# razayunus/ManhattanSLAM

Hardware: AMD Instinct MI355X
Metric: RGB-D frames/sec at 640x480 (ORB+surfel front end) (higher is better)
Workload: dtype u8/i32 (ORB)/f32+f64 (surfel)

## Files before the change

### manhattanslam_amd/csrc/msl_sf.h

```cpp
#pragma once

#include "msl_common.h"

#include <hip/hip_ext.h>

namespace msl {
namespace sf {

constexpr int SP = 8;
constexpr int NCHUNK = 10;
constexpr double MAX_ANGLE_COS = 0.1, HUBER_RANGE = 0.4, MIN_TOLERATE_DIFF = 0.1;
constexpr unsigned T_INF = 0xFFFFFFFFu;
constexpr int PROP_ROUNDS = 6;
constexpr unsigned short IDX_NONE = 0xFFFF, IDX_PLANE = 0xFFFE;
constexpr int LIST_D = 256;
constexpr int SCAN_ITEMS = 1024;
#ifndef MSL_SUB_ITEMS
#define MSL_SUB_ITEMS 128
#endif
constexpr int SUB_ITEMS = MSL_SUB_ITEMS;
constexpr int DEFER_WIN = 32;
#ifndef MSL_FUSEREC_PLANES
#define MSL_FUSEREC_PLANES 0
#endif
__host__ __device__ inline size_t fuserec_index(int nseeds, unsigned seed, int word) {
#if MSL_FUSEREC_PLANES
    return (size_t)word * (size_t)nseeds + seed;
#else
    (void)nseeds; return 3 * (size_t)seed + (size_t)word;
#endif
}

enum SfCtr {
    CTR_LIVE = 0,
    CTR_NEW = 1,
    CTR_DELETED = 2,
    CTR_UPDATED = 3,
    CTR_BEFORE = 4,
    CTR_ERR = 5,
    CTR_AFTER = 6,
    CTR_TAIL_FLAG = 7,
    CTR_SELECTED = 7,
    CTR_TOT_NEW = 8, CTR_TOT_DELETED = 9, CTR_TOT_UPDATED = 10, CTR_TOT_KF = 11, CTR_TOT_BEFORE = 12,
    CTR_WIDE = 13,
    CTR_COUNT = 16
};

struct alignas(16) HotPk { float px, py, pz; unsigned tl; };
struct HotRec { float px, py, pz; int updateTimes, lastUpdate; };
constexpr unsigned HOT_WIDE = 0x80000000u, HOT_HOLE = 0xFFFFFFFFu;
__host__ __device__ inline bool tl_fits(int ut, int lu) { return (unsigned)ut < 2048u && ((unsigned)lu + (1u << 19)) < (1u << 20); }
__host__ __device__ inline unsigned tl_pack(int ut, int lu) { return ((unsigned)ut << 20) | ((unsigned)lu & 0xFFFFFu); }
__host__ __device__ inline int tl_ut(unsigned tl) { return (int)(tl >> 20); }
__host__ __device__ inline int tl_lu(unsigned tl) { return (int)(tl << 12) >> 12; }
struct alignas(32) ColdRec { float nx, ny, nz, size, color, weight; unsigned rgbf; unsigned _spare; };
constexpr unsigned COLD_WIDE = 1u << 24;
struct MapSoA {
    HotPk *hot;
    ColdRec *cold;
    int *rgbWide;
    int *utlWide;
    long long *wideFlag;
};
__host__ __device__ inline bool rgb_fits(int r, int g, int b) { return ((unsigned)r | (unsigned)g | (unsigned)b) < 256u; }
__host__ __device__ inline unsigned rgb_pack(int r, int g, int b) { return (unsigned)r | ((unsigned)g << 8) | ((unsigned)b << 16); }

template <typename T> using gptr = const T __attribute__((address_space(1))) *;
struct FrameDev {
    const uint8_t *gray; const float *depth; const int32_t *member;
    float pose[16], invPose[16];
    int ref, _pad;
#ifdef __HIPCC__
    __device__ __forceinline__ gptr<uint8_t> grayG() const { return (gptr<uint8_t>)gray; }
    __device__ __forceinline__ gptr<float> depthG() const { return (gptr<float>)depth; }
    __device__ __forceinline__ gptr<int32_t> memberG() const { return (gptr<int32_t>)member; }
#endif
};

struct alignas(32) AssignRec {
    float x, y, meanIntensity;
    unsigned stable;
    double invDepth;
    unsigned long long _pad;
};

struct FuseAux {
    MapSoA map;
    unsigned long long cap;
    unsigned *delU, *delUCount;
    unsigned *delList;
};
struct DeferCtl {
    long long ext[DEFER_WIN + 1];
    unsigned delCnt[DEFER_WIN];
    unsigned logBase[DEFER_WIN];
    unsigned nMoves;
    int flagStride;
    const uint8_t *candOk, *fused;
    const msl_surfel *cand;
    FuseAux aux;
};

struct SfDev {
    int W, H, spW, spH, nseeds, npx;
    float fx, fy, cx, cy, fuseFar, fuseNear;
    unsigned long long gstride, gbytes, dstride, mstride;
    unsigned gsB, dsB, msB;
    const FrameDev *frames;
    msl_seed *seeds, *seedsTmp;
    msl_surfel *cand;
    uint8_t *candOk;
    uint8_t *fused;
    uint2 *tex;
    float4 *fuseRec;
    unsigned short *index, *amap;
    unsigned *tmin;
    AssignRec *arec;
    float *pxInv;
    unsigned *wl;
    unsigned *wlCount;
    int *chunkAbort;
    int *changed;
    MapSoA map;
    unsigned long long cap;
    long long *ctr;
    msl_surfel *newSurfels;
    unsigned *blockSums, *blockUpd, *delList, *srcOf;
    unsigned *sbKeys, *deal;
    int dealG;
    unsigned *tickets;
    unsigned *delU;
    unsigned *delUCount;
    const float *colX, *rowY;
    int pxStride;
    int flagStride;
    int kf;
    int prevSlotAbs;
    DeferCtl *dc;
    unsigned *moveDst;
    unsigned long long *loc64;
    unsigned *vposD;
    unsigned *locKeys, *vposKeys;
    unsigned *dBig;
    unsigned *bitmap;
    HotPk *stageHot; ColdRec *stageCold; int *stageRgb, *stageUtl;
};

#ifdef __HIPCC__
__device__ __forceinline__ AssignRec assign_rec(const msl_seed &s) {
    AssignRec a;
    a.x = s.x; a.y = s.y; a.meanIntensity = s.meanIntensity; a.stable = s.stable ? 1u : 0u;
    a.invDepth = s.meanDepth > 0 ? 1.0 / (double)s.meanDepth : -1.0; a._pad = 0;
    return a;
}
__device__ __forceinline__ int seed_chunk(int seedI, int nseeds) {
    const int step = nseeds / NCHUNK;
    if (step == 0) return NCHUNK - 1;
    const int c = seedI / step;
    return c > NCHUNK - 1 ? NCHUNK - 1 : c;
}
template <typename T> __device__ __forceinline__ gptr<T> byte_off(gptr<T> p, unsigned off) {
    return reinterpret_cast<gptr<T>>(reinterpret_cast<const char __attribute__((address_space(1))) *>(p) + off);
}
template <typename T> __device__ __forceinline__ gptr<T> byte_off(const T *p, unsigned off) { return byte_off((gptr<T>)p, off); }
template <typename T> using gptr_w = T __attribute__((address_space(1))) *;
template <typename T> __device__ __forceinline__ gptr_w<T> byte_off_w(T *p, unsigned off) {
    return reinterpret_cast<gptr_w<T>>(reinterpret_cast<char __attribute__((address_space(1))) *>((gptr_w<T>)p) + off);
}
__device__ __forceinline__ uint8_t gray_at(const SfDev &P, const FrameDev &F, int y, int x) { return *byte_off(F.grayG(), (unsigned)y * P.gsB + (unsigned)x); }
__device__ __forceinline__ float depth_at(const SfDev &P, const FrameDev &F, int y, int x) { return *byte_off(F.depthG(), (unsigned)y * P.dsB + 4u * (unsigned)x); }
__device__ __forceinline__ int32_t member_at(const SfDev &P, const FrameDev &F, int y, int x) {
    return *byte_off(F.memberG(), ((unsigned)y >> 1) * P.msB + 4u * ((unsigned)x >> 1));
}
__device__ __forceinline__ void vec3b(const SfDev &P, const FrameDev &F, float row, float col, int &r, int &g, int &b) {
    const unsigned long long off = (unsigned long long)(int)row * P.gstride + 3ull * (unsigned long long)(int)col;
    r = off < P.gbytes ? F.grayG()[off] : 0;
    g = off + 1 < P.gbytes ? F.grayG()[off + 1] : 0;
    b = off + 2 < P.gbytes ? F.grayG()[off + 2] : 0;
}
__device__ __forceinline__ void back_project(const SfDev &P, float u, float v, float d, float &x, float &y, float &z) {
    x = (u - P.cx) / P.fx * d;
    y = (v - P.cy) / P.fy * d;
    z = d;
}
__device__ __forceinline__ float get_weight(float d) { const double a = 1.0 / (double)d / (double)d; return (float)(1.0 < a ? 1.0 : a); }
__device__ __forceinline__ void mul4(const float *m, float v0, float v1, float v2, float v3, float out[4]) {
#pragma unroll
    for (int r = 0; r < 4; r++) out[r] = ((m[r] * v0 + m[4 + r] * v1) + m[8 + r] * v2) + m[12 + r] * v3;
}
__device__ __forceinline__ void mul3(const float *m, float v0, float v1, float v2, float out[3]) {
#pragma unroll
    for (int r = 0; r < 3; r++) out[r] = (m[r] * v0 + m[4 + r] * v1) + m[8 + r] * v2;
}
#endif

template <typename T>
__host__ __device__ inline void inverse4(const T *m, T *inv) {
#define M_(r, c) m[(c) * 4 + (r)]
#define DET3(r0, r1, r2, c0, c1, c2)                                                                     \
    (M_(r0, c0) * (M_(r1, c1) * M_(r2, c2) - M_(r1, c2) * M_(r2, c1)) -                                 \
     M_(r0, c1) * (M_(r1, c0) * M_(r2, c2) - M_(r1, c2) * M_(r2, c0)) +                                 \
     M_(r0, c2) * (M_(r1, c0) * M_(r2, c1) - M_(r1, c1) * M_(r2, c0)))
    T cof[4][4];
    for (int r = 0; r < 4; r++)
        for (int c = 0; c < 4; c++) {
            int rr[3], cc[3], k = 0;
            for (int i = 0; i < 4; i++) if (i != r) rr[k++] = i;
            k = 0;
            for (int i = 0; i < 4; i++) if (i != c) cc[k++] = i;
            const T d = DET3(rr[0], rr[1], rr[2], cc[0], cc[1], cc[2]);
            cof[r][c] = ((r + c) & 1) ? -d : d;
        }
    const T det = ((M_(0, 0) * cof[0][0] + M_(0, 1) * cof[0][1]) + M_(0, 2) * cof[0][2]) + M_(0, 3) * cof[0][3];
    for (int r = 0; r < 4; r++)
        for (int c = 0; c < 4; c++) inv[c * 4 + r] = cof[c][r] / det;
#undef DET3
#undef M_
}

#ifdef __HIPCC__
__device__ __forceinline__ bool xcd_slot(int blocksPerFrame, int nSlots, int &slot, int &blk) {
    const unsigned lin = blockIdx.x;
    const unsigned j = lin >> 3;
    slot = (int)(lin & 7u) + 8 * (int)(j / (unsigned)blocksPerFrame);
    blk = (int)(j % (unsigned)blocksPerFrame);
    return slot < nSlots;
}
#endif
inline unsigned xcd_grid(int blocksPerFrame, int nSlots) { return 8u * (unsigned)((nSlots + 7) / 8) * (unsigned)blocksPerFrame; }

enum { SK_SEED_INIT = 0, SK_ASSIGN, SK_PROP, SK_COMMIT_PX, SK_UPDATE_SEEDS, SK_COMMIT_SEEDS, SK_SEED_PLANE, SK_FUSE, SK_NEW, SK_COMPACT,
       SK_CONVERT, SK_COPY };

#define MSL_SF_LAUNCH_LDS(prof, kid, st, kern, grid, block, lds, ...)                                  \
    do {                                                                                               \
        hipEvent_t _ea, _eb;                                                                           \
        if ((prof).kernel_pair(kid, &_ea, &_eb))                                                       \
            hipExtLaunchKernelGGL(kern, grid, block, lds, st, _ea, _eb, 0, __VA_ARGS__);               \
        else                                                                                           \
            hipLaunchKernelGGL(kern, grid, block, lds, st, __VA_ARGS__);                               \
    } while (0)
#define MSL_SF_LAUNCH(prof, kid, st, kern, grid, block, ...) MSL_SF_LAUNCH_LDS(prof, kid, st, kern, grid, block, 0, __VA_ARGS__)

bool sp_init_attributes(int nseeds);
void sp_launch_stage(KernelProfiler &prof, hipStream_t st, const SfDev &P, int nFrames, bool propLds);
void sp_launch_depth_u16(hipStream_t st, const void *src, size_t srcStride, size_t srcFrameStride, float *dst, size_t dstFrameStride, int W, int H, int nFrames,
                         float factor);
int sp_debug_div100(const float *x_host, double *out_host, size_t n);
int sp_debug_chain(const float *x_host, const int32_t *n_host, int lists, int huber, float *out_host);
void map_launch_fuse(KernelProfiler &prof, hipStream_t st, const SfDev &P, int slot, const FrameDev &F, int nSubGrid, int nSubHint, bool deferred, bool dealt, unsigned blkStride);
void map_launch_compact(KernelProfiler &prof, hipStream_t st, const SfDev &P, int slot, bool resident);
void map_launch_deal(hipStream_t st, const SfDev &P);
int map_debug_deal(const uint32_t *keys_host, int G, uint32_t *deal_host);
void map_launch_replay(KernelProfiler &prof, hipStream_t st, const SfDev &P, int nFrames, unsigned blkStride);
void map_launch_empty_pair(KernelProfiler &prof, hipStream_t st);
void map_launch_set_ctr(hipStream_t st, const SfDev &P, long long n, int wide);
void map_launch_add_ctr(hipStream_t st, const SfDev &P, long long add);
void map_launch_aos_to_soa(KernelProfiler &prof, hipStream_t st, const SfDev &P, const msl_surfel *src, long long n, bool atEnd);
void map_launch_soa_to_aos(KernelProfiler &prof, hipStream_t st, const SfDev &P, msl_surfel *dst, long long n);
void map_launch_select_count(hipStream_t st, const SfDev &P, int mode, int arg);
void map_launch_select_write(hipStream_t st, const SfDev &P, int mode, int arg, msl_surfel *out, int markDeleted);
void map_launch_collect_changed(hipStream_t st, const SfDev &P, int ref, long long n, unsigned *count, unsigned *idxOut, msl_surfel *recOut, unsigned capOut);
void map_launch_empty(hipStream_t st, int grid, hipEvent_t a, hipEvent_t b);

}
}
```

### manhattanslam_amd/csrc/msl_sf_compact.hip

```cpp

#include "msl_sf_map_dev.h"

namespace {
template <int NT>
__device__ __forceinline__ void deal_subblocks(const unsigned *keys, int G, unsigned *deal, unsigned *s_hist, unsigned *s_off, unsigned *s_wave, unsigned *s_aux) {
    static_assert(NT == 256, "one histogram bin per thread");
    const unsigned t = threadIdx.x;
    constexpr int CH = 32 * NT;
    auto load_pack = [&](int base, unsigned (&kp)[8]) {
        uint4 v[8];
#pragma unroll
        for (int q = 0; q < 8; q++) v[q] = *reinterpret_cast<const uint4 *>(keys + base + 32 * (int)t + 4 * q);
#pragma unroll
        for (int q = 0; q < 8; q++) kp[q] = min(v[q].x, 255u) | (min(v[q].y, 255u) << 8) | (min(v[q].z, 255u) << 16) | (min(v[q].w, 255u) << 24);
    };
    auto next_word = [&](unsigned (&kp)[8]) -> unsigned {
        const unsigned w = kp[0];
#pragma unroll
        for (int q = 0; q < 7; q++) kp[q] = kp[q + 1];
        kp[7] = w;
        return w;
    };
    auto count_chunk = [&](int base, unsigned (&kp)[8], bool hist) -> unsigned {
        unsigned fc = 0;
#pragma unroll 1
        for (int d = 0; d < 8; d++) {
            const unsigned w = next_word(kp);
#pragma unroll
            for (int b = 0; b < 4; b++) {
                const unsigned key = (w >> (8 * b)) & 255u;
                const bool in = base + 32 * (int)t + 4 * d + b < G;
                if (hist && in && key != 255u) atomicAdd(&s_hist[key], 1u);
                fc += in && key == 255u ? 1u : 0u;
            }
        }
        return fc;
    };
    unsigned k0[8];
    load_pack(0, k0);
    s_hist[t] = 0;
    __syncthreads();
    const unsigned fc0 = count_chunk(0, k0, true);
    for (int base = CH; base < G; base += CH) { unsigned kc[8]; load_pack(base, kc); (void)count_chunk(base, kc, true); }
    __syncthreads();
    unsigned NI, fTot0, ex, fb0;
    block_excl_scan_pair(t < 255u ? s_hist[t] : 0u, fc0, s_wave, &NI, &fTot0, ex, fb0);
    const unsigned gs = (unsigned)G >> 3;
    auto inS = [&](unsigned x) { return (x * NI + 7u) >> 3; };
    auto outS = [&](unsigned x) { return x * gs - inS(x); };
    {
        unsigned x0 = 0;
#pragma unroll
        for (unsigned y = 1; y < 8; y++) x0 += ex >= inS(y) ? 1u : 0u;
        s_off[t] = ex - inS(x0);
        s_hist[t] = x0 | ((inS(x0 + 1) - inS(x0)) << 3);
        if (t < 9) s_aux[t] = inS(t);
    }
    __syncthreads();
    unsigned fillBase = 0;
    auto place_chunk = [&](int base, unsigned (&kp)[8], unsigned fb, unsigned ftot) {
        fb += fillBase;
        fillBase += ftot;
        unsigned xf = 0;
#pragma unroll
        for (unsigned y = 1; y < 8; y++) xf += fb >= outS(y) ? 1u : 0u;
        unsigned jf = (inS(xf + 1) - inS(xf)) + (fb - outS(xf));
#pragma unroll 1
        for (int d = 0; d < 8; d++) {
            const unsigned w = next_word(kp);
            unsigned rr[4], tb[4];
#pragma unroll
            for (int b = 0; b < 4; b++) {
                const unsigned key = (w >> (8 * b)) & 255u;
                rr[b] = 0; tb[b] = 0;
                if (base + 32 * (int)t + 4 * d + b < G && key != 255u) { rr[b] = atomicAdd(&s_off[key], 1u); tb[b] = s_hist[key]; }
            }
#pragma unroll
            for (int b = 0; b < 4; b++) {
                const unsigned key = (w >> (8 * b)) & 255u;
                const int sb = base + 32 * (int)t + 4 * d + b;
                const bool in = sb < G, iv = in && key != 255u, fl = in && key == 255u;
                unsigned x = tb[b] & 7u, room = tb[b] >> 3, j = rr[b];
                if (__builtin_expect(__ballot((iv && j >= room) || (fl && jf >= gs)) != 0ull, 0)) {
                    if (iv) while (j >= room) { j -= room; x++; room = s_aux[x + 1] - s_aux[x]; }
                    if (fl) while (jf >= gs) { xf++; jf = s_aux[xf + 1] - s_aux[xf]; }
                }
                const unsigned at = (iv ? x : xf) * gs + (iv ? j : jf);
                if (in) deal[at] = (unsigned)sb;
                jf += fl ? 1u : 0u;
            }
        }
    };
    place_chunk(0, k0, fb0, fTot0);
    for (int base = CH; base < G; base += CH) {
        unsigned kc[8];
        load_pack(base, kc);
        const unsigned fc = count_chunk(base, kc, false);
        unsigned ftot;
        const unsigned fb = block_excl_scan(fc, s_wave, &ftot);
        place_chunk(base, kc, fb, ftot);
    }
    __syncthreads();
}
__global__ __launch_bounds__(256) void k_deal(const unsigned *keys, int G, unsigned *deal) {
    __shared__ unsigned s_hist[256], s_off[256], s_wave[33], s_aux[16];
    deal_subblocks<256>(keys, G, deal, s_hist, s_off, s_wave, s_aux);
}

constexpr int TAIL_MAX_HOPS = 64;


constexpr int SMALL_D = 512, SMALL_CHUNKS = 48;

struct CompactArgs {
    int nseeds, flagStride, dealG, _pad;
    unsigned long long cap;
    MapSoA map;
    long long *ctr;
    const uint8_t *candOk, *fused;
    const msl_surfel *cand;
    msl_surfel *newSurfels;
    unsigned *blockSums, *blockUpd, *delList, *srcOf, *tickets, *delU, *delUCount;
    const unsigned *sbKeys; unsigned *deal;
};
__host__ inline CompactArgs compact_args(const SfDev &P, int slot) {
    CompactArgs A;
    A.nseeds = P.nseeds; A.flagStride = P.flagStride; A.dealG = P.dealG; A._pad = 0; A.cap = P.cap; A.map = P.map; A.ctr = P.ctr;
    A.candOk = P.candOk + (size_t)slot * P.flagStride; A.fused = P.fused + (size_t)slot * P.flagStride; A.cand = P.cand + (size_t)slot * P.nseeds;
    A.newSurfels = P.newSurfels; A.blockSums = P.blockSums; A.blockUpd = P.blockUpd; A.delList = P.delList; A.srcOf = P.srcOf; A.tickets = P.tickets;
    A.delU = P.delU; A.delUCount = P.delUCount; A.sbKeys = P.sbKeys; A.deal = P.deal;
    return A;
}

template <int NQW>
__global__ __launch_bounds__(256) void k_compact(CompactArgs P, int mode) {
    constexpr int NT = 256, TILE = 4 * NT;
    __shared__ unsigned s_wave[33];
    __shared__ unsigned s_dl[SMALL_D];
    __shared__ unsigned s_raw[LIST_D];
    __shared__ unsigned s_last, s_upd, s_nzChunks, s_base, s_cntChunk;
    __shared__ unsigned s_nzIdx[SMALL_CHUNKS], s_nzCnt[SMALL_CHUNKS], s_nzSortIdx[SMALL_CHUNKS], s_nzSortCnt[SMALL_CHUNKS];
    __shared__ int s_fallback;
    __builtin_amdgcn_s_setprio(3);
    if (mode == 0 && blockIdx.x == 1 && P.dealG > 0) deal_subblocks<NT>(P.sbKeys, P.dealG, P.deal, s_raw, s_dl, s_wave, s_nzIdx);
    if (mode == 0 && blockIdx.x != 0 && *P.delUCount <= LIST_D) return;
    const uint4 bs0 = *reinterpret_cast<const uint4 *>(P.blockSums + 4 * threadIdx.x);
    constexpr int NBU = 8;
    uint4 bu[NBU];
#pragma unroll
    for (int q = 0; q < NBU; q++) bu[q] = *reinterpret_cast<const uint4 *>(P.blockUpd + TILE * q + 4 * threadIdx.x);
    static_assert(LIST_D == NT, "one hand-over entry per thread");
    const unsigned du = P.delU[threadIdx.x];
    const unsigned dHand = *P.delUCount;
    const long long n = P.ctr[CTR_LIVE];
    const bool bad = P.ctr[CTR_ERR] == 20;
    const uint8_t *candOk = P.candOk, *fused = P.fused;
    const int per = (((P.nseeds + NT - 1) / NT) + 3) & ~3;
    const int s0 = threadIdx.x * per, s1 = min(s0 + per, P.nseeds);
    unsigned cnt = 0;
    unsigned long long emit = 0, emitHi = 0;
    const msl_surfel *cand = P.cand;
    const bool aligned4 = (P.nseeds & 3) == 0 && ((reinterpret_cast<size_t>(candOk) | reinterpret_cast<size_t>(fused)) & 3) == 0;
    auto flags_in_one_trip = [&](auto nqTag) {
        constexpr int NQ = decltype(nqTag)::value;
        unsigned cw[NQ], fw[NQ];
#pragma unroll
        for (int q = 0; q < NQ; q++) {
            const int i = s0 + 4 * q;
            const bool in = 4 * q < per && i < s1;
            cw[q] = in ? *reinterpret_cast<const unsigned *>(candOk + i) : 0u;
            fw[q] = in ? *reinterpret_cast<const unsigned *>(fused + i) : 0u;
        }
#pragma unroll
        for (int q = 0; q < NQ; q += 8)
            asm volatile("" ::"v"(cw[q]), "v"(cw[q + 1]), "v"(cw[q + 2]), "v"(cw[q + 3]), "v"(cw[q + 4]), "v"(cw[q + 5]), "v"(cw[q + 6]), "v"(cw[q + 7]),
                         "v"(fw[q]), "v"(fw[q + 1]), "v"(fw[q + 2]), "v"(fw[q + 3]), "v"(fw[q + 4]), "v"(fw[q + 5]), "v"(fw[q + 6]), "v"(fw[q + 7]));
#pragma unroll
        for (int q = 0; q < NQ; q++)
#pragma unroll
            for (int j = 0; j < 4; j++) {
                const unsigned e = (s0 + 4 * q + j < s1 && ((cw[q] >> (8 * j)) & 0xFF) && !((fw[q] >> (8 * j)) & 0xFF)) ? 1u : 0u;
                cnt += e;
                if (4 * q + j < 64) emit |= (unsigned long long)e << ((4 * q + j) & 63);
                else emitHi |= (unsigned long long)e << ((4 * q + j - 64) & 63);
            }
    };
    if constexpr (NQW > 0) {
        (void)aligned4;
        flags_in_one_trip(std::integral_constant<int, NQW>{});
    } else {
        for (int i = s0; i < s1; i += 4) {
            unsigned c4, f4;
            if (i + 4 <= P.nseeds && ((reinterpret_cast<size_t>(candOk + i) | reinterpret_cast<size_t>(fused + i)) & 3) == 0) {
                c4 = *reinterpret_cast<const unsigned *>(candOk + i); f4 = *reinterpret_cast<const unsigned *>(fused + i);
            } else {
                c4 = f4 = 0;
                for (int j = 0; j < 4 && i + j < P.nseeds; j++) { c4 |= (unsigned)candOk[i + j] << (8 * j); f4 |= (unsigned)fused[i + j] << (8 * j); }
            }
#pragma unroll
            for (int j = 0; j < 4; j++) {
                const unsigned e = (i + j < s1 && ((c4 >> (8 * j)) & 0xFF) && !((f4 >> (8 * j)) & 0xFF)) ? 1u : 0u;
                cnt += e;
                if (i + j - s0 < 64) emit |= (unsigned long long)e << (i + j - s0);
                else if (i + j - s0 < 128) emitHi |= (unsigned long long)e << (i + j - s0 - 64);
            }
        }
    }
    const long long nblk = (n + SUB_ITEMS - 1) / SUB_ITEMS;
    const long long nWg = nblk;
    unsigned updPart = 0;
#pragma unroll
    for (int q = 0; q < NBU; q++) {
        const long long c = TILE * q + 4 * threadIdx.x;
        updPart += (c < nWg ? bu[q].x : 0u) + (c + 1 < nWg ? bu[q].y : 0u) + (c + 2 < nWg ? bu[q].z : 0u) + (c + 3 < nWg ? bu[q].w : 0u);
    }
    s_raw[threadIdx.x] = du;
    if (threadIdx.x == 0) { s_upd = 0; s_fallback = 0; s_nzChunks = 0; }
    __syncthreads();
    const bool fastest = mode == 0 && dHand <= LIST_D;
    unsigned vsum = 0;
    if (!fastest)
        for (long long t0 = 0; t0 < nblk; t0 += TILE) {
            const long long c = t0 + 4 * threadIdx.x;
            const uint4 v4 = t0 == 0 ? bs0 : *reinterpret_cast<const uint4 *>(P.blockSums + c);
            const unsigned x[4] = {c < nblk ? v4.x : 0u, c + 1 < nblk ? v4.y : 0u, c + 2 < nblk ? v4.z : 0u, c + 3 < nblk ? v4.w : 0u};
#pragma unroll
            for (int j = 0; j < 4; j++)
                if (x[j] > 0) {
                    vsum += x[j];
                    const unsigned q = atomicAdd(&s_nzChunks, 1u);
                    if (q < SMALL_CHUNKS) { s_nzIdx[q] = (unsigned)(c + j); s_nzCnt[q] = x[j]; }
                }
        }
    unsigned Dtot, Ku, exUnused, pos;
    block_excl_scan_pair(vsum, cnt, s_wave, &Dtot, &Ku, exUnused, pos);
    const long long D = fastest ? (long long)dHand : (long long)Dtot;
    const bool small = mode == 0 && !fastest && D <= SMALL_D && s_nzChunks <= SMALL_CHUNKS;
    const bool single = fastest || small;
    if (single && blockIdx.x != 0) return;
    if (mode == 0 && !bad) {
        if (fastest) {
            if (threadIdx.x < D) {
                unsigned r = 0;
                for (unsigned j = 0; j < (unsigned)D; j++) r += s_raw[j] < du ? 1u : 0u;
                s_dl[r] = du;
            }
        } else if (small) {
            const unsigned nz = s_nzChunks;
            if (threadIdx.x < nz) {
                const unsigned me = s_nzIdx[threadIdx.x];
                unsigned r = 0;
                for (unsigned j = 0; j < nz; j++) r += s_nzIdx[j] < me ? 1u : 0u;
                s_nzSortIdx[r] = me; s_nzSortCnt[r] = s_nzCnt[threadIdx.x];
            }
            __syncthreads();
            unsigned base = 0;
            for (unsigned it = 0; it < nz; it++) {
                const long long i0 = (long long)s_nzSortIdx[it] * SUB_ITEMS + threadIdx.x;
                const unsigned f = (threadIdx.x < (unsigned)SUB_ITEMS && i0 < n && hot_is_deleted(P.map, i0)) ? 1u : 0u;
                unsigned tt;
                const unsigned w = base + block_excl_scan(f, s_wave, &tt);
                if (f) s_dl[w] = (unsigned)i0;
                base += s_nzSortCnt[it];
            }
        } else {
            unsigned carry = 0;
            for (long long t0 = 0; t0 < nblk; t0 += TILE) {
                const long long c = t0 + 4 * threadIdx.x;
                const uint4 v4 = t0 == 0 ? bs0 : *reinterpret_cast<const uint4 *>(P.blockSums + c);
                const unsigned v[4] = {c < nblk ? v4.x : 0u, c + 1 < nblk ? v4.y : 0u, c + 2 < nblk ? v4.z : 0u, c + 3 < nblk ? v4.w : 0u};
                unsigned tot;
                const unsigned ex = carry + block_excl_scan(v[0] + v[1] + v[2] + v[3], s_wave, &tot);
                const long long nIter = (min(t0 + TILE, nblk) - t0 - blockIdx.x + gridDim.x - 1) / gridDim.x;
                for (long long it = 0; it < nIter; it++) {
                    const long long b = t0 + blockIdx.x + it * gridDim.x;
                    const int q = (int)(b - t0);
                    if ((int)threadIdx.x == (q >> 2)) {
                        const int comp = q & 3;
                        s_base = ex + (comp > 0 ? v[0] : 0u) + (comp > 1 ? v[1] : 0u) + (comp > 2 ? v[2] : 0u);
                        s_cntChunk = v[comp];
                    }
                    __syncthreads();
                    const unsigned base = s_base, cntChunk = s_cntChunk;
                    if (cntChunk == 0) { __syncthreads(); continue; }
                    const long long i0 = b * SUB_ITEMS + threadIdx.x;
                    const unsigned f = (threadIdx.x < (unsigned)SUB_ITEMS && i0 < n && hot_is_deleted(P.map, i0)) ? 1u : 0u;
                    unsigned tt;
                    const unsigned w = base + block_excl_scan(f, s_wave, &tt);
                    if (f) st_agent(&P.delList[w], (unsigned)i0);
                }
                carry += tot;
                __syncthreads();
            }
        }
    }
    __syncthreads();
    if (mode == 0 && !single && !last_workgroup(&P.tickets[1], &s_last)) return;
    {
        unsigned u = updPart;
        for (long long c2 = (long long)NBU * TILE + threadIdx.x; c2 < nWg; c2 += blockDim.x) u += P.blockUpd[c2];
        u = wave_incl_scan(u);
        if ((threadIdx.x & 63) == 63 && u) atomicAdd(&s_upd, u);
    }
    const long long K = Ku;
    const long long nAfter = mode == 1 ? n : (D >= K ? n - (D - K) : n + (K - D));
    const bool place = mode == 0 && !bad && (unsigned long long)nAfter <= P.cap;
    auto DL = [&](long long j) -> unsigned { return single ? s_dl[j] : ld_agent(&P.delList[j]); };
    if (cnt) {
        auto emit_one = [&](const msl_surfel &e) {
            const long long k = pos++;
            P.newSurfels[k] = e;
            if (place)
                store_surfel(P.map, k < D ? (long long)DL(D - 1 - k) : n + (k - D), e);
        };
        for (unsigned long long m = emit; m; m &= m - 1) emit_one(cand[s0 + __builtin_ctzll(m)]);
        for (unsigned long long mh = emitHi; mh; mh &= mh - 1) emit_one(cand[s0 + 64 + __builtin_ctzll(mh)]);
        for (int i = s0 + 128; i < s1; i++)
            if (candOk[i] && !fused[i]) emit_one(cand[i]);
    }
    __syncthreads();
    if (threadIdx.x == 0) {
        P.ctr[CTR_NEW] = K; P.ctr[CTR_DELETED] = D; P.ctr[CTR_UPDATED] = s_upd; P.ctr[CTR_BEFORE] = n; P.ctr[CTR_AFTER] = nAfter;
        P.ctr[CTR_TOT_NEW] += K; P.ctr[CTR_TOT_DELETED] += D; P.ctr[CTR_TOT_UPDATED] += s_upd; P.ctr[CTR_TOT_KF] += 1; P.ctr[CTR_TOT_BEFORE] += n;
        if ((unsigned long long)nAfter > P.cap) P.ctr[CTR_ERR] = 20;
    }
    if (!place) { if (threadIdx.x == 0) *P.delUCount = 0; return; }
    const long long t0 = threadIdx.x, stride = blockDim.x;
    if (D > K) {
        const long long R = D - K, nFinal = n - R;
        auto lower = [&](long long x) -> long long {
            long long lo = 0, hi = R;
            while (lo < hi) { const long long mid = (lo + hi) >> 1; if ((long long)DL(mid) < x) lo = mid + 1; else hi = mid; }
            return lo;
        };
        const long long cntLow = lower(nFinal);
        for (long long a = t0; a < cntLow; a += stride) {
            long long p = nFinal + a;
            int hop = 0;
            for (; hop < TAIL_MAX_HOPS; hop++) {
                const long long lb = lower(p);
                if (lb < R && (long long)DL(lb) == p) p = n - (R - lb);
                else break;
            }
            if (hop == TAIL_MAX_HOPS) s_fallback = 1;
            P.srcOf[a] = (unsigned)p;
        }
        __syncthreads();
        if (s_fallback) {
            if (threadIdx.x == 0)
                for (long long i = 1; i <= R; i++) {
                    const long long hole = DL(R - i), src = n - i;
                    if (src != hole) move_surfel(P.map, hole, src);
                }
        } else {
            for (long long a = t0; a < cntLow; a += stride) move_surfel(P.map, (long long)DL(a), (long long)P.srcOf[a]);
        }
    }
    if (threadIdx.x == 0) { P.ctr[CTR_LIVE] = nAfter; *P.delUCount = 0; }
}
}

namespace msl {
namespace sf {
void map_launch_compact(KernelProfiler &prof, hipStream_t st, const SfDev &P, int slot, bool resident) {
    const CompactArgs A = compact_args(P, slot);
    const int per = (((P.nseeds + 255) / 256) + 3) & ~3;
    const bool aligned4 = (P.nseeds & 3) == 0 && ((reinterpret_cast<size_t>(A.candOk) | reinterpret_cast<size_t>(A.fused)) & 3) == 0;
    const dim3 grid(resident ? 128 : 1);
    if (per <= 32 && aligned4) MSL_SF_LAUNCH(prof, SK_COMPACT, st, k_compact<8>, grid, dim3(256), A, resident ? 0 : 1);
    else if (per <= 96 && aligned4) MSL_SF_LAUNCH(prof, SK_COMPACT, st, k_compact<24>, grid, dim3(256), A, resident ? 0 : 1);
    else MSL_SF_LAUNCH(prof, SK_COMPACT, st, k_compact<0>, grid, dim3(256), A, resident ? 0 : 1);
}
void map_launch_deal(hipStream_t st, const SfDev &P) { hipLaunchKernelGGL(k_deal, dim3(1), dim3(256), 0, st, P.sbKeys, P.dealG, P.deal); }
int map_debug_deal(const uint32_t *keys_host, int G, uint32_t *deal_host) {
    if (!keys_host || !deal_host || G < 8 || (G & 7)) return MSL_ERR_INVALID;
    const size_t pad = (size_t)G + 8192;
    DevBuf keys, deal;
    MSL_HIP_TRY(grow_all(0, {{keys, sizeof(unsigned) * pad}, {deal, sizeof(unsigned) * (G + 64)}}));
    unsigned *dk = (unsigned *)keys.p, *dd = (unsigned *)deal.p;
    MSL_HIP_TRY(hipMemset(dk, 0xFF, sizeof(unsigned) * pad)); MSL_HIP_TRY(hipMemset(dd, 0xFF, sizeof(unsigned) * G));
    MSL_HIP_TRY(hipMemcpy(dk, keys_host, sizeof(unsigned) * G, hipMemcpyHostToDevice));
    hipLaunchKernelGGL(k_deal, dim3(1), dim3(256), 0, 0, dk, G, dd);
    MSL_HIP_TRY(hipGetLastError());
    MSL_HIP_TRY(hipMemcpy(deal_host, dd, sizeof(unsigned) * G, hipMemcpyDeviceToHost));
    return MSL_OK;
}
}
}
```

### manhattanslam_amd/csrc/msl_sf_debug.hip

```cpp

#include "msl_sf_handle.h"

#include <vector>

using namespace msl;
using namespace msl::sf;

namespace {
const char *kSfNames[MSL_SF_NKERNELS] = {"kb_seed_init", "kb_assign", "kb_prop", "kb_commit_px", "kb_update_seeds", "kb_commit_seeds",
                                         "kb_seed_plane", "k_fuse", "k_empty", "k_compact", "k_convert", "copy"};
}

extern "C" {

int msl_sf_debug_seeds(msl_sf *h, msl_seed *out) noexcept {
    try {
    if (!h || !out) return MSL_ERR_INVALID;
    MSL_HIP_TRY(hipSetDevice(h->device));
    int rc = sync_all(h);
    if (rc != MSL_OK) return rc;
    const size_t ns = h->dev.nseeds;
    MSL_HIP_TRY(hipMemcpy(out, h->dev.seeds + ns * h->lastSlot, sizeof(msl_seed) * ns, hipMemcpyDeviceToHost));
    std::vector<uint8_t> fused(ns);
    MSL_HIP_TRY(hipMemcpy(fused.data(), h->dev.fused + (size_t)h->dev.flagStride * h->lastSlot, ns, hipMemcpyDeviceToHost));
    for (size_t i = 0; i < ns; i++) out[i].fused = fused[i] & 1;
    return MSL_OK;
    } MSL_ABI_CATCH_INT
}
int msl_sf_debug_ctr(msl_sf *h, int64_t out[16]) noexcept {
    try {
    if (!h || !out) return MSL_ERR_INVALID;
    MSL_HIP_TRY(hipSetDevice(h->device));
    int rc = read_ctr(h);
    if (rc != MSL_OK) return rc;
    static_assert(CTR_COUNT == 16, "msl_sf_debug_ctr hands out every counter");
    for (int i = 0; i < CTR_COUNT; i++) out[i] = host_ctr(h, (SfCtr)i);
    return MSL_OK;
    } MSL_ABI_CATCH_INT
}
int msl_sf_debug_scratch(msl_sf *h, int which, size_t offset_words, uint32_t *out, size_t n_words) noexcept {
    try {
    if (!h || !out || which < 0 || which > 5) return MSL_ERR_INVALID;
    if (which == 5) {
        if (n_words < 2) return MSL_ERR_INVALID;
        out[0] = (uint32_t)h->kfClassic; out[1] = (uint32_t)h->kfDeferred;
        return MSL_OK;
    }
    if (which == 4) {
        if (n_words < 1) return MSL_ERR_INVALID;
        out[0] = (uint32_t)h->dealG;
        return MSL_OK;
    }
    if (offset_words + n_words > (which < 2 ? h->dev.cap : h->blkStride)) return MSL_ERR_INVALID;
    MSL_HIP_TRY(hipSetDevice(h->device));
    int rc = sync_all(h);
    if (rc != MSL_OK) return rc;
    const uint32_t *src = which == 0 ? h->dev.srcOf : which == 1 ? h->dev.delList : which == 2 ? h->dev.sbKeys : h->dev.deal;
    MSL_HIP_TRY(hipMemcpy(out, src + offset_words, sizeof(uint32_t) * n_words, hipMemcpyDeviceToHost));
    return MSL_OK;
    } MSL_ABI_CATCH_INT
}
int msl_sf_debug_event_overhead(msl_sf *h, int grid, int n, float *mean_us) noexcept {
    try {
    if (!h || !mean_us || n < 1 || grid < 1) return MSL_ERR_INVALID;
    MSL_HIP_TRY(hipSetDevice(h->device));
    int rc = sync_all(h);
    if (rc != MSL_OK) return rc;
    std::vector<hipEvent_t> ev(2 * (size_t)n);
    for (auto &e : ev) MSL_HIP_TRY(hipEventCreate(&e));
    for (int i = 0; i < n; i++) map_launch_empty(h->mapStream, grid, ev[2 * i], ev[2 * i + 1]);
    MSL_HIP_TRY(hipStreamSynchronize(h->mapStream));
    double tot = 0;
    for (int i = 0; i < n; i++) { float ms = 0; MSL_HIP_TRY(hipEventElapsedTime(&ms, ev[2 * i], ev[2 * i + 1])); tot += ms; }
    for (auto &e : ev) (void)hipEventDestroy(e);
    *mean_us = (float)(tot * 1e3 / n);
    return MSL_OK;
    } MSL_ABI_CATCH_INT
}
int msl_sf_debug_index(msl_sf *h, int32_t *out) noexcept {
    try {
    if (!h || !out) return MSL_ERR_INVALID;
    MSL_HIP_TRY(hipSetDevice(h->device));
    int rc = sync_all(h);
    if (rc != MSL_OK) return rc;
    const size_t npx = h->dev.npx;
    std::vector<unsigned short> tmp(npx);
    MSL_HIP_TRY(hipMemcpy(tmp.data(), h->dev.index + (size_t)h->dev.pxStride * h->lastSlot, sizeof(unsigned short) * npx, hipMemcpyDeviceToHost));
    for (size_t i = 0; i < npx; i++) out[i] = tmp[i];
    return MSL_OK;
    } MSL_ABI_CATCH_INT
}

int msl_debug_deal(const uint32_t *keys_host, int n_subblocks, uint32_t *deal_host) noexcept { try { return map_debug_deal(keys_host, n_subblocks, deal_host); } MSL_ABI_CATCH_INT }
int msl_debug_div100(const float *x_host, double *out_host, size_t n) noexcept { try { return sp_debug_div100(x_host, out_host, n); } MSL_ABI_CATCH_INT }
int msl_debug_chain_sum(const float *x_host, const int32_t *n_host, int lists, int huber, float *out_host) noexcept { try { return sp_debug_chain(x_host, n_host, lists, huber, out_host); } MSL_ABI_CATCH_INT }
const char *msl_sf_kernel_name(int k) noexcept { try { return (k >= 0 && k < MSL_SF_NKERNELS) ? kSfNames[k] : ""; } MSL_ABI_CATCH_PTR }

}
```

### manhattanslam_amd/csrc/msl_sf_fuse.hip

```cpp

#include "msl_sf_map_dev.h"

namespace {
__device__ __forceinline__ void mul4r(const float *m, float v0, float v1, float v2, float v3, float out[3]) {
#pragma unroll
    for (int r = 0; r < 3; r++) out[r] = ((m[r] * v0 + m[3 + r] * v1) + m[6 + r] * v2) + m[9 + r] * v3;
}
__device__ __forceinline__ void mul3r(const float *m, float v0, float v1, float v2, float out[3]) {
#pragma unroll
    for (int r = 0; r < 3; r++) out[r] = (m[r] * v0 + m[3 + r] * v1) + m[6 + r] * v2;
}

template <bool DEFER, bool spawnWave>
__device__ __forceinline__ void fuse_body(const FuseArgs &P, const FuseFrame &F, int nSubHint, unsigned waveIdx, int G) {
    constexpr int KPL = SUB_ITEMS / 64;
    constexpr long long WSPAN = 64 * KPL;
    struct { HotPk *hot; ColdRec *cold; } M = {P.hot, P.cold};
    const FuseAux *aux = &P.dc->aux;
    const unsigned lane0 = threadIdx.x;
    const uint2 *tex = P.tex;
    const float4 *fuseRec = P.fuseRec;
    uint8_t *fused = P.fused;
    const int ref = F.ref;
    const float cameraF = (float)(((double)fabsf(P.fx) + (double)fabsf(P.fy)) / 2.0);
    const float halfF = 0.5f * cameraF;
    const bool pending = DEFER && P.kf > 0;
    long long E0v = 0;
    if (pending) E0v = P.dc->ext[P.kf - 1];
    long long E0 = 0;
    if (DEFER && spawnWave) E0 = ((long long)__builtin_amdgcn_readfirstlane((int)(E0v >> 32)) << 32) | (unsigned)__builtin_amdgcn_readfirstlane((int)E0v);
    if (spawnWave && !pending) return;
    if (DEFER && !pending && waveIdx == 0 && lane0 == 0) P.dc->ext[0] = P.ctr[CTR_LIVE];
    if (DEFER && !spawnWave && waveIdx == 0 && lane0 == 0) P.dc->logBase[P.kf] = P.kf > 0 ? P.dc->logBase[P.kf - 1] + P.dc->delCnt[P.kf - 1] : 0u;
    unsigned spK = 0;
    if (DEFER && spawnWave) {
        unsigned excl;
        spK = spawn_count(P, lane0, excl);
        if (lane0 == 0) P.dc->ext[P.kf] = E0 + (long long)spK;
        if (spK == 0) return;
    }
#ifndef MSL_FUSE_CHUNK
#define MSL_FUSE_CHUNK 16
#endif
    constexpr unsigned FUSE_CHUNK = MSL_FUSE_CHUNK;
    long long sb0;
    if (!spawnWave && P.deal != nullptr) {
        const unsigned gs = (unsigned)G >> 3;
        const unsigned *dp = P.deal + ((waveIdx & 7u) * gs + (waveIdx >> 3));
        unsigned dv;
        asm volatile("s_load_dword %0, %1, 0x0\n\ts_waitcnt lgkmcnt(0)" : "=s"(dv) : "s"(dp) : "memory");
        sb0 = (long long)dv;
    } else {
        long long lin = waveIdx;
        constexpr unsigned T = 8u * FUSE_CHUNK;
        const unsigned full = ((unsigned)G / T) * T;
        if (waveIdx < full) { const unsigned grp = waveIdx / T, r = waveIdx % T; lin = (long long)grp * T + (r & 7u) * FUSE_CHUNK + (r >> 3); }
        sb0 = (long long)G - 1 - lin;
    }
    for (long long it = 0;; it++) {
        unsigned lane = lane0;
        asm volatile("" : "+v"(lane));
#define REC_LOCAL(k) (64u * (unsigned)(k) + lane)
        const long long sb = sb0 + it * G;
        long long c0, n = 0, cntIdx;
        if (DEFER && spawnWave) {
            c0 = E0 + it * WSPAN;
            n = E0 + (long long)spK;
            if (c0 >= n) return;
            unsigned excl;
            (void)spawn_count(P, lane, excl);
            emit_records(P, E0, c0, KPL, lane, spK, excl);
            cntIdx = E0 / SUB_ITEMS + 1 + it;
        } else {
            c0 = sb * WSPAN; cntIdx = sb;
            if (pending) {
                if (it > 0) {
                    E0 = ((long long)__builtin_amdgcn_readfirstlane((int)(E0v >> 32)) << 32) | (unsigned)__builtin_amdgcn_readfirstlane((int)E0v);
                    if (c0 >= E0) return;
                }
            } else if (sb >= nSubHint && c0 >= __hip_atomic_load(&P.ctr[CTR_LIVE], __ATOMIC_RELAXED, __HIP_MEMORY_SCOPE_AGENT)) return;
        }
        HotPk hq[KPL];
#pragma unroll
        for (int k = 0; k < KPL; k++) hq[k] = M.hot[c0 + REC_LOCAL(k)];
        if (!pending) n = P.ctr[CTR_LIVE];
        else if (!spawnWave) {
            E0 = ((long long)__builtin_amdgcn_readfirstlane((int)(E0v >> 32)) << 32) | (unsigned)__builtin_amdgcn_readfirstlane((int)E0v);
            if (c0 >= E0) return;
            n = E0;
        }
        unsigned stp = 0;
        unsigned keyAcc = 0;
        float pzv[KPL];
        unsigned offT[KPL];
        unsigned anyTl = 0;
#pragma unroll
        for (int k = 0; k < KPL; k++) anyTl |= hq[k].tl;
        const bool anyHi = __builtin_expect(__ballot(anyTl >> 31) != 0ull, 0);
#pragma unroll
        for (int k = 0; k < KPL; k++) {
            const long long i = c0 + REC_LOCAL(k);
            const float x = hq[k].px, y = hq[k].py, z = hq[k].pz;
            const unsigned tl = hq[k].tl;
            int ut = tl_ut(tl), lu = tl_lu(tl);
            bool hole = false;
            if (anyHi) {
                if (tl == HOT_WIDE) { const int *w = aux->map.utlWide; ut = w[2 * i]; lu = w[2 * i + 1]; }
                else if (tl & 0x80000000u) hole = true;
            }
            float pc[3];
            mul4r(F.inv, x, y, z, 1.0f, pc);
            const bool inRange = !(pc[2] < P.fuseNear || pc[2] > P.fuseFar);
            const bool live = i < n && !hole, stale = ref - lu > 5 && ut < 5;
            int st = 0;
            if (live) st = stale ? (ut != 0 ? 1 : 2) : (ut == 0 ? 2 : 0);
            const bool cand = live && !stale && ut != 0 && inRange;
            unsigned off = 0;
            {
                const float zq = inRange ? pc[2] : 1.0f;
                const float projectU = pc[0] * P.fx / zq + P.cx, projectV = pc[1] * P.fy / zq + P.cy;
                const int pUInt = round_half_up_pixel(projectU), pVInt = round_half_up_pixel(projectV);
                const bool inImage = !(pUInt < 1 || pUInt > P.W - 2 || pVInt < 1 || pVInt > P.H - 2);
                if (cand && inImage) { st = 3; keyAcc += (((unsigned)pVInt * (unsigned)P.rowScale) >> 16) | 0x10000u; }
                off = st == 3 ? (unsigned)(pVInt * P.W + pUInt) : 0u;
            }
            stp |= (unsigned)st << (2 * k); pzv[k] = pc[2];
            offT[k] = off;
        }
        uint2 tx[KPL];
        {
#pragma unroll
            for (int k = 0; k < KPL; k++) tx[k] = tex[offT[k]];
            if constexpr (KPL == 4) asm volatile("" ::"v"(tx[0].x), "v"(tx[1].x), "v"(tx[2].x), "v"(tx[3].x), "v"(tx[0].y), "v"(tx[1].y), "v"(tx[2].y), "v"(tx[3].y));
            else asm volatile("" ::"v"(tx[0].x), "v"(tx[KPL - 1].x), "v"(tx[0].y), "v"(tx[KPL - 1].y));
        }
        if (!(DEFER && spawnWave)) {
            const unsigned ks = (unsigned)__builtin_amdgcn_readlane((int)wave_incl_scan(keyAcc), 63);
            const unsigned kc = ks >> 16;
            const unsigned key = kc ? min((unsigned)((float)(ks & 0xFFFFu) * __builtin_amdgcn_rcpf((float)kc)), 254u) : 255u;
            if (lane == 0) P.sbKeys[cntIdx] = key;
        }
        unsigned fl = 0;
        unsigned cntDel = 0;
#pragma unroll
        for (int k = 0; k < KPL; k++) {
            const unsigned st = (stp >> (2 * k)) & 3u;
            const bool occluded = st == 3u && (double)pzv[k] < (double)__uint_as_float(tx[k].x) - 1.0;
            const bool del = st == 1u || st == 2u || occluded;
            if (DEFER) { if (del) M.hot[c0 + REC_LOCAL(k)].tl = HOT_HOLE; }
            else if (st == 1u || occluded) {
                if (__builtin_expect(hq[k].tl == HOT_WIDE, 0)) aux->map.utlWide[2 * (c0 + REC_LOCAL(k))] = 0;
                else M.hot[c0 + REC_LOCAL(k)].tl = hq[k].tl & 0xFFFFFu;
            }
            fl |= del ? (1u << k) : 0u;
            fl |= (st == 3u && !occluded) ? (16u << k) : 0u;
            cntDel += (unsigned)__popcll(__ballot(del));
        }
        auto list_base = [&](unsigned c) -> unsigned {
            unsigned base = 0, prior = 0;
            if (DEFER && P.kf > 0) prior = P.dc->logBase[P.kf - 1] + P.dc->delCnt[P.kf - 1];
            if (lane == 0) base = atomicAdd(P.delCount, c);
            return (unsigned)__builtin_amdgcn_readfirstlane((int)base) + prior;
        };
        auto hand_over = [&](bool d, unsigned long long m, unsigned base, long long i) {
            if (d) {
                const unsigned j = base + lane_rank(m);
                if (DEFER || j < (unsigned)LIST_D) P.delOut[j] = (unsigned)i;
            }
        };
        if (cntDel) {
            unsigned base = list_base(cntDel);
#pragma unroll
            for (int k = 0; k < KPL; k++) {
                const bool d = (fl >> k) & 1u;
                const unsigned long long m = __ballot(d);
                hand_over(d, m, base, c0 + REC_LOCAL(k)); base += (unsigned)__popcll(m);
            }
        }
        unsigned rcv[KPL], bk[KPL];
        unsigned total = 0;
#pragma unroll
        for (int k = 0; k < KPL; k++) {
            const bool sv = (fl >> (4 + k)) & 1u;
            const unsigned long long m = __ballot(sv);
            const unsigned c = (unsigned)__popcll(m), rs = lane_rank(m);
            const unsigned dest = (sv ? total + rs : total + c + (lane - rs)) & 63u;
            const unsigned payload = sv ? (REC_LOCAL(k) | 0x100u | (tx[k].y << 16)) : 0u;
            rcv[k] = (unsigned)__builtin_amdgcn_ds_permute((int)(dest * 4u), (int)payload);
            bk[k] = total;
            total += c;
        }
        const unsigned rounds = (total + 63u) >> 6;
        unsigned nupd = 0, cntDelB = 0;
        for (unsigned r = 0; r < rounds; r++) {
            unsigned item = 0u;
#pragma unroll
            for (int k = 0; k < KPL; k++) {
                const unsigned rk = (bk[k] + ((lane - bk[k]) & 63u)) >> 6;
                if ((rcv[k] & 0x100u) && rk == r) item = rcv[k];
            }
            const long long i = c0 + (item & 0xFFu);
            const unsigned sp = item >> 16;
            const HotPk h = M.hot[i];
            ColdRec c;
            {
                const float4 cn = *reinterpret_cast<const float4 *>(M.cold + i);
                c.nx = cn.x; c.ny = cn.y; c.nz = cn.z; c.size = cn.w; c.weight = M.cold[i].weight;
            }
            const float4 f0 = fuseRec[fuserec_index(P.nseeds, sp, 0)], f1 = fuseRec[fuserec_index(P.nseeds, sp, 1)], f2 = fuseRec[fuserec_index(P.nseeds, sp, 2)];
            const float *poseM = F.frame->pose;
            const float r00 = poseM[0], r10 = poseM[1], r20 = poseM[2], r01 = poseM[4], r11 = poseM[5], r21 = poseM[6], r02 = poseM[8], r12 = poseM[9], r22 = poseM[10];
            asm volatile("" ::"v"(h.px), "v"(h.tl), "v"(c.nx), "v"(c.weight), "v"(f0.x), "v"(f1.x), "v"(f2.x), "v"(r00), "v"(r01), "v"(r02));
            bool upd = false, delB = false;
            if (item && __float_as_uint(f2.w) != 0u) {
                const float seedDepth = f0.w;
                const float pz = ((F.inv[2] * h.px + F.inv[5] * h.py) + F.inv[8] * h.pz) + F.inv[11] * 1.0f;
                float tolerateDiff = (pz * pz) / halfF * 4.0f;
                tolerateDiff = tolerateDiff < MIN_TOLERATE_DIFF ? (float)MIN_TOLERATE_DIFF : tolerateDiff;
                if (!(pz < seedDepth - tolerateDiff) && !(pz > seedDepth + tolerateDiff)) {
                    float nc[3];
                    mul3r(F.inv, c.nx, c.ny, c.nz, nc);
                    const float normDiffCos = nc[0] * f0.x + nc[1] * f0.y + nc[2] * f0.z;
                    if (normDiffCos < MAX_ANGLE_COS) {
                        if (DEFER) M.hot[i].tl = HOT_HOLE;
                        else if (__builtin_expect(h.tl == HOT_WIDE, 0)) aux->map.utlWide[2 * i] = 0;
                        else M.hot[i].tl = h.tl & 0xFFFFFu;
                        delB = true;
                    } else {
                        const float oldWeight = c.weight;
                        const float newWeight = f1.w;
                        const float sumWeight = oldWeight + newWeight;
                        const float fusedPx = (h.px * oldWeight + newWeight * f1.x) / sumWeight;
                        const float fusedPy = (h.py * oldWeight + newWeight * f1.y) / sumWeight;
                        const float fusedPz = (h.pz * oldWeight + newWeight * f1.z) / sumWeight;
                        float fusedNx = nc[0] * oldWeight + newWeight * f0.x;
                        float fusedNy = nc[1] * oldWeight + newWeight * f0.y;
                        float fusedNz = nc[2] * oldWeight + newWeight * f0.z;
                        const float newNormLength = sqrtf(fusedNx * fusedNx + fusedNy * fusedNy + fusedNz * fusedNz);
                        fusedNx = fusedNx / newNormLength; fusedNy = fusedNy / newNormLength; fusedNz = fusedNz / newNormLength;
                        float newNormW[3];
                        newNormW[0] = (r00 * fusedNx + r01 * fusedNy) + r02 * fusedNz;
                        newNormW[1] = (r10 * fusedNx + r11 * fusedNy) + r12 * fusedNz;
                        newNormW[2] = (r20 * fusedNx + r21 * fusedNy) + r22 * fusedNz;
                        int ut = (int)(h.tl >> 20);
                        if (__builtin_expect(h.tl == HOT_WIDE, 0)) ut = aux->map.utlWide[2 * i];
                        unsigned tlNew = tl_pack(ut + 1, ref);
                        if (__builtin_expect(!tl_fits(ut + 1, ref), 0)) {
                            int *w = aux->map.utlWide;
                            w[2 * i] = ut + 1; w[2 * i + 1] = ref;
                            asm volatile("" ::: "memory");
                            set_wide_flag_ptr(aux->map.wideFlag, 2ull);
                            tlNew = HOT_WIDE;
                        }
                        c.rgbf = __float_as_uint(f2.z);
                        c.nx = newNormW[0]; c.ny = newNormW[1]; c.nz = newNormW[2];
                        c.weight = sumWeight;
                        c.color = f2.y;
                        const float newSize = f2.x;
                        if (newSize < c.size) c.size = newSize;
                        u32x4 hv = {__float_as_uint(fusedPx), __float_as_uint(fusedPy), __float_as_uint(fusedPz), tlNew};
                        u32x4 c0v = {__float_as_uint(c.nx), __float_as_uint(c.ny), __float_as_uint(c.nz), __float_as_uint(c.size)};
                        u32x4 c1v = {__float_as_uint(c.color), __float_as_uint(c.weight), c.rgbf, 0u};
                        st16(M.hot + i, hv);
                        st16(M.cold + i, c0v);
                        st16(reinterpret_cast<u32x4 *>(M.cold + i) + 1, c1v);
                        fused[sp] = 1;
                        upd = true;
                    }
                }
            }
            nupd += (unsigned)__popcll(__ballot(upd));
            const unsigned long long mb = __ballot(delB);
            if (mb) {
                const unsigned cb = (unsigned)__popcll(mb);
                hand_over(delB, mb, list_base(cb), i);
                cntDelB += cb;
            }
        }
        if (lane == 0) {
            if (!DEFER) P.blockSums[cntIdx] = cntDel + cntDelB;
            P.blockUpd[cntIdx] = nupd;
        }
        if (!(DEFER && spawnWave) && (sb + G) * WSPAN >= n) return;
    }
#undef REC_LOCAL
}

template <bool DEFER>
__global__ __launch_bounds__(64) __attribute__((amdgpu_waves_per_eu(6, 8))) void k_fuse(FuseArgs P, FuseFrame F, int nSubHint) {
    __builtin_amdgcn_s_setprio(3);
    if (DEFER) {
        if (blockIdx.x == 0) fuse_body<DEFER, true>(P, F, nSubHint, 0u, (int)gridDim.x - 1);
        else fuse_body<DEFER, false>(P, F, nSubHint, blockIdx.x - 1u, (int)gridDim.x - 1);
    } else {
        fuse_body<false, false>(P, F, nSubHint, blockIdx.x, (int)gridDim.x);
    }
}
}

namespace msl {
namespace sf {
void map_launch_fuse(KernelProfiler &prof, hipStream_t st, const SfDev &P, int slot, const FrameDev &F, int nSubGrid, int nSubHint, bool deferred, bool dealt, unsigned blkStride) {
    const FuseArgs A = fuse_args(P, slot, deferred, blkStride, dealt);
    const FuseFrame FF = fuse_frame(F, P.frames + slot);
    if (deferred) MSL_SF_LAUNCH(prof, SK_FUSE, st, k_fuse<true>, dim3((unsigned)nSubGrid + 1u), dim3(64), A, FF, nSubHint);
    else MSL_SF_LAUNCH(prof, SK_FUSE, st, k_fuse<false>, dim3((unsigned)nSubGrid), dim3(64), A, FF, nSubHint);
}
}
}
```

### manhattanslam_amd/csrc/msl_sf_map.hip

```cpp

#include "msl_sf_map_dev.h"

namespace {
__device__ __forceinline__ bool select_pred(const HotRec &h, int mode, int arg) {
    return mode == 0 ? (h.updateTimes > 0 && h.lastUpdate == arg) : (h.updateTimes >= arg);
}
__global__ __launch_bounds__(256) void k_select_count(SfDev P, int mode, int arg) {
    __shared__ unsigned s_c;
    const long long n = P.ctr[CTR_LIVE];
    const long long nblk = (n + SCAN_ITEMS - 1) / SCAN_ITEMS;
    for (long long b = blockIdx.x; b < nblk; b += gridDim.x) {
        if (threadIdx.x == 0) s_c = 0;
        __syncthreads();
        unsigned c = 0;
        for (int k = 0; k < SCAN_ITEMS / 256; k++) {
            const long long i = b * SCAN_ITEMS + k * 256 + threadIdx.x;
            if (i < n && select_pred(hot_load(P.map, i), mode, arg)) c++;
        }
        if (c) atomicAdd(&s_c, c);
        __syncthreads();
        if (threadIdx.x == 0) P.blockSums[b] = s_c;
        __syncthreads();
    }
}
__global__ __launch_bounds__(1024) void k_select_scan(SfDev P) {
    __shared__ unsigned s_wave[17];
    const long long n = P.ctr[CTR_LIVE];
    const int nblk = (int)((n + SCAN_ITEMS - 1) / SCAN_ITEMS);
    unsigned carry = 0;
    for (int b0 = 0; b0 < nblk; b0 += 1024) {
        const int b = b0 + threadIdx.x;
        const unsigned v = b < nblk ? P.blockSums[b] : 0;
        unsigned tot;
        const unsigned ex = carry + block_excl_scan(v, s_wave, &tot);
        if (b < nblk) P.blockSums[b] = ex;
        carry += tot;
    }
    if (threadIdx.x == 0) P.ctr[CTR_SELECTED] = carry;
}
__global__ __launch_bounds__(256) void k_select_write(SfDev P, int mode, int arg, msl_surfel *out, int markDeleted) {
    __shared__ unsigned s_wave[17];
    const long long n = P.ctr[CTR_LIVE];
    const long long nblk = (n + SCAN_ITEMS - 1) / SCAN_ITEMS;
    for (long long b = blockIdx.x; b < nblk; b += gridDim.x) {
        unsigned base = P.blockSums[b];
        for (int k = 0; k < SCAN_ITEMS / 256; k++) {
            const long long i = b * SCAN_ITEMS + k * 256 + threadIdx.x;
            HotRec h{};
            unsigned tl = 0;
            if (i < n) { tl = P.map.hot[i].tl; h = hot_load(P.map, i); }
            const bool sel = i < n && select_pred(h, mode, arg);
            unsigned tot;
            const unsigned pos = base + block_excl_scan(sel ? 1u : 0u, s_wave, &tot);
            if (sel) {
                msl_surfel e;
                load_surfel(P.map, i, h, e);
                out[pos] = e;
                if (markDeleted) hot_mark_deleted(P.map, i, tl);
            }
            base += tot;
        }
    }
}
__global__ void k_add_ctr(long long *ctr, long long add) {
    if (threadIdx.x == 0) { ctr[CTR_LIVE] += add; ctr[CTR_BEFORE] = ctr[CTR_LIVE]; ctr[CTR_AFTER] = ctr[CTR_LIVE]; }
}
__global__ __launch_bounds__(256) void k_aos_to_soa_at(MapSoA M, const msl_surfel *src, long long n, const long long *ctr) {
    const long long i = (long long)blockIdx.x * 256 + threadIdx.x;
    if (i < n) store_surfel(M, ctr[CTR_LIVE] + i, src[i]);
}

__global__ __launch_bounds__(256) void k_aos_to_soa(MapSoA M, const msl_surfel *src, long long n) {
    const long long i = (long long)blockIdx.x * 256 + threadIdx.x;
    if (i < n) store_surfel(M, i, src[i]);
}
__global__ __launch_bounds__(256) void k_soa_to_aos(MapSoA M, msl_surfel *dst, long long n) {
    const long long i = (long long)blockIdx.x * 256 + threadIdx.x;
    if (i >= n) return;
    const HotRec h = hot_load(M, i);
    msl_surfel e;
    load_surfel(M, i, h, e);
    dst[i] = e;
}
__global__ void k_set_ctr(long long *ctr, long long n, unsigned *delUCount, int wide) {
    if (threadIdx.x == 0) {
        delUCount[0] = 0;
        ctr[CTR_LIVE] = n; ctr[CTR_NEW] = 0; ctr[CTR_DELETED] = 0; ctr[CTR_UPDATED] = 0; ctr[CTR_BEFORE] = n; ctr[CTR_AFTER] = n; ctr[CTR_TAIL_FLAG] = 0;
        if (wide >= 0) ctr[CTR_WIDE] = wide;
    }
}

__global__ __launch_bounds__(64) void k_collect_changed(SfDev P, int ref, long long n, unsigned *count, unsigned *idxOut, msl_surfel *recOut, unsigned capOut) {
    const long long sb = blockIdx.x;
    if (!(P.blockSums[sb] | P.blockUpd[sb])) return;
    const unsigned lane = threadIdx.x;
    for (int k = 0; k < SUB_ITEMS / 64; k++) {
        const long long i = sb * SUB_ITEMS + k * 64 + lane;
        HotRec h; h.px = h.py = h.pz = 0; h.updateTimes = 1; h.lastUpdate = ref - 1;
        if (i < n) h = hot_load(P.map, i);
        const bool ch = i < n && (h.updateTimes == 0 || h.lastUpdate == ref);
        const unsigned long long m = __ballot(ch);
        if (!m) continue;
        unsigned base = 0;
        if (lane == 0) base = atomicAdd(count, (unsigned)__popcll(m));
        base = __builtin_amdgcn_readfirstlane(base);
        if (ch) {
            const unsigned j = base + lane_rank(m);
            if (j < capOut) { msl_surfel e; load_surfel(P.map, i, h, e); recOut[j] = e; idxOut[j] = (unsigned)i; }
        }
    }
}

__global__ void k_empty(int grid_dummy) { (void)grid_dummy; }
}

namespace msl {
namespace sf {
void map_launch_empty_pair(KernelProfiler &prof, hipStream_t st) {
    hipEvent_t ea, eb;
    if (prof.kernel_pair(SK_NEW, &ea, &eb)) hipExtLaunchKernelGGL(k_empty, dim3(1), dim3(64), 0, st, ea, eb, 0, 0);
}
void map_launch_set_ctr(hipStream_t st, const SfDev &P, long long n, int wide) { hipLaunchKernelGGL(k_set_ctr, dim3(1), dim3(64), 0, st, P.ctr, n, P.delUCount, wide); }
void map_launch_add_ctr(hipStream_t st, const SfDev &P, long long add) { hipLaunchKernelGGL(k_add_ctr, dim3(1), dim3(64), 0, st, P.ctr, add); }
void map_launch_aos_to_soa(KernelProfiler &prof, hipStream_t st, const SfDev &P, const msl_surfel *src, long long n, bool atEnd) {
    if (atEnd) hipLaunchKernelGGL(k_aos_to_soa_at, dim3((unsigned)((n + 255) / 256)), dim3(256), 0, st, P.map, src, n, P.ctr);
    else MSL_SF_LAUNCH(prof, SK_CONVERT, st, k_aos_to_soa, dim3((unsigned)((n + 255) / 256)), dim3(256), P.map, src, n);
}
void map_launch_soa_to_aos(KernelProfiler &prof, hipStream_t st, const SfDev &P, msl_surfel *dst, long long n) {
    MSL_SF_LAUNCH(prof, SK_CONVERT, st, k_soa_to_aos, dim3((unsigned)((n + 255) / 256)), dim3(256), P.map, dst, n);
}
void map_launch_select_count(hipStream_t st, const SfDev &P, int mode, int arg) {
    hipLaunchKernelGGL(k_select_count, dim3(512), dim3(256), 0, st, P, mode, arg);
    hipLaunchKernelGGL(k_select_scan, dim3(1), dim3(1024), 0, st, P);
}
void map_launch_select_write(hipStream_t st, const SfDev &P, int mode, int arg, msl_surfel *out, int markDeleted) {
    hipLaunchKernelGGL(k_select_write, dim3(512), dim3(256), 0, st, P, mode, arg, out, markDeleted);
}
void map_launch_collect_changed(hipStream_t st, const SfDev &P, int ref, long long n, unsigned *count, unsigned *idxOut, msl_surfel *recOut, unsigned capOut) {
    const unsigned nblk = (unsigned)((n + SUB_ITEMS - 1) / SUB_ITEMS);
    hipLaunchKernelGGL(k_collect_changed, dim3(nblk), dim3(64), 0, st, P, ref, n, count, idxOut, recOut, capOut);
}
void map_launch_empty(hipStream_t st, int grid, hipEvent_t a, hipEvent_t b) { hipExtLaunchKernelGGL(k_empty, dim3((unsigned)grid), dim3(64), 0, st, a, b, 0, grid); }
}
}
```

### manhattanslam_amd/csrc/msl_sf_map_dev.h

```cpp
#pragma once

#include "msl_sf.h"

#ifdef __HIPCC__

using namespace msl;
using namespace msl::sf;

namespace {

__device__ __forceinline__ unsigned ld_agent(const unsigned *p) { return __hip_atomic_load(p, __ATOMIC_RELAXED, __HIP_MEMORY_SCOPE_AGENT); }
__device__ __forceinline__ void st_agent(unsigned *p, unsigned v) { __hip_atomic_store(p, v, __ATOMIC_RELAXED, __HIP_MEMORY_SCOPE_AGENT); }
__device__ __forceinline__ unsigned long long ld_agent64(const unsigned long long *p) { return __hip_atomic_load(p, __ATOMIC_RELAXED, __HIP_MEMORY_SCOPE_AGENT); }
__device__ __forceinline__ void st_agent64(unsigned long long *p, unsigned long long v) { __hip_atomic_store(p, v, __ATOMIC_RELAXED, __HIP_MEMORY_SCOPE_AGENT); }

__device__ __forceinline__ void set_wide_flag_ptr(long long *flag, unsigned long long bit) { atomicOr(reinterpret_cast<unsigned long long *>(flag), bit); }
__device__ __forceinline__ void set_wide_flag(const MapSoA &M, unsigned long long bit) { set_wide_flag_ptr(M.wideFlag, bit); }
__device__ __forceinline__ void tl_unpack(const MapSoA &M, long long i, unsigned tl, int &ut, int &lu) {
    ut = tl_ut(tl); lu = tl_lu(tl);
    if (tl & 0x80000000u) {
        if (tl == HOT_WIDE) { ut = M.utlWide[2 * i]; lu = M.utlWide[2 * i + 1]; }
        else { ut = 0; lu = 0; }
    }
}
__device__ __forceinline__ HotRec hot_load(const MapSoA &M, long long i) {
    const HotPk p = M.hot[i];
    HotRec h; h.px = p.px; h.py = p.py; h.pz = p.pz;
    tl_unpack(M, i, p.tl, h.updateTimes, h.lastUpdate);
    return h;
}
__device__ __forceinline__ unsigned tl_store_word(const MapSoA &M, long long i, int ut, int lu) {
    if (tl_fits(ut, lu)) return tl_pack(ut, lu);
    M.utlWide[2 * i] = ut; M.utlWide[2 * i + 1] = lu;
    set_wide_flag(M, 2ull);
    return HOT_WIDE;
}
__device__ __forceinline__ void hot_store(const MapSoA &M, long long i, const HotRec &h) {
    HotPk p; p.px = h.px; p.py = h.py; p.pz = h.pz; p.tl = tl_store_word(M, i, h.updateTimes, h.lastUpdate);
    M.hot[i] = p;
}
__device__ __forceinline__ void hot_mark_deleted(const MapSoA &M, long long i, unsigned tl) {
    if (tl == HOT_WIDE) M.utlWide[2 * i] = 0;
    else M.hot[i].tl = tl & 0xFFFFFu;
}
__device__ __forceinline__ bool hot_is_deleted(const MapSoA &M, long long i) {
    const unsigned tl = M.hot[i].tl;
    return tl == HOT_WIDE ? M.utlWide[2 * i] == 0 : (tl == HOT_HOLE || (tl >> 20) == 0);
}

struct ColdBits { uint4 a, b; };
__device__ __forceinline__ ColdRec cold_load(const ColdRec *p) {
    const uint4 *q = reinterpret_cast<const uint4 *>(p);
    ColdBits v; v.a = q[0]; v.b = q[1];
    ColdRec c;
    c.nx = __uint_as_float(v.a.x); c.ny = __uint_as_float(v.a.y); c.nz = __uint_as_float(v.a.z); c.size = __uint_as_float(v.a.w);
    c.color = __uint_as_float(v.b.x); c.weight = __uint_as_float(v.b.y); c.rgbf = v.b.z; c._spare = v.b.w;
    return c;
}
__device__ __forceinline__ void cold_store(ColdRec *p, const ColdRec &c) {
    uint4 *q = reinterpret_cast<uint4 *>(p);
    q[0] = make_uint4(__float_as_uint(c.nx), __float_as_uint(c.ny), __float_as_uint(c.nz), __float_as_uint(c.size));
    q[1] = make_uint4(__float_as_uint(c.color), __float_as_uint(c.weight), c.rgbf, c._spare);
}

__device__ __forceinline__ void store_surfel(const MapSoA &M, long long i, const msl_surfel &e) {
    HotRec h; h.px = e.px; h.py = e.py; h.pz = e.pz; h.updateTimes = e.updateTimes; h.lastUpdate = e.lastUpdate;
    ColdRec c; c.nx = e.nx; c.ny = e.ny; c.nz = e.nz; c.size = e.size; c.color = e.color; c.weight = e.weight; c._spare = 0;
    if (rgb_fits(e.r, e.g, e.b)) c.rgbf = rgb_pack(e.r, e.g, e.b);
    else { c.rgbf = COLD_WIDE; set_wide_flag(M, 1ull); M.rgbWide[3 * i] = e.r; M.rgbWide[3 * i + 1] = e.g; M.rgbWide[3 * i + 2] = e.b; }
    hot_store(M, i, h); cold_store(M.cold + i, c);
}
__device__ __forceinline__ void load_surfel(const MapSoA &M, long long i, const HotRec &h, msl_surfel &e) {
    const ColdRec c = cold_load(M.cold + i);
    e.px = h.px; e.py = h.py; e.pz = h.pz; e.nx = c.nx; e.ny = c.ny; e.nz = c.nz; e.size = c.size; e.color = c.color;
    if (c.rgbf & COLD_WIDE) { e.r = M.rgbWide[3 * i]; e.g = M.rgbWide[3 * i + 1]; e.b = M.rgbWide[3 * i + 2]; }
    else { e.r = (int)(c.rgbf & 255u); e.g = (int)((c.rgbf >> 8) & 255u); e.b = (int)((c.rgbf >> 16) & 255u); }
    e.weight = c.weight; e.updateTimes = h.updateTimes; e.lastUpdate = h.lastUpdate;
}
__device__ __forceinline__ void move_surfel(const MapSoA &M, long long dst, long long src) {
    const ColdRec c = cold_load(M.cold + src);
    const HotPk p = M.hot[src];
    M.hot[dst] = p; cold_store(M.cold + dst, c);
    if (p.tl == HOT_WIDE) { M.utlWide[2 * dst] = M.utlWide[2 * src]; M.utlWide[2 * dst + 1] = M.utlWide[2 * src + 1]; }
    if (c.rgbf & COLD_WIDE) { M.rgbWide[3 * dst] = M.rgbWide[3 * src]; M.rgbWide[3 * dst + 1] = M.rgbWide[3 * src + 1]; M.rgbWide[3 * dst + 2] = M.rgbWide[3 * src + 2]; }
}

__device__ __forceinline__ bool last_workgroup(unsigned *ticket, unsigned *s_flag) {
    asm volatile("s_waitcnt vmcnt(0)" ::: "memory");
    __syncthreads();
    if (threadIdx.x == 0) {
        const unsigned t = atomicAdd(ticket, 1u);
        *s_flag = (t == gridDim.x - 1) ? 1u : 0u;
        if (*s_flag) __hip_atomic_store(ticket, 0u, __ATOMIC_RELAXED, __HIP_MEMORY_SCOPE_AGENT);
    }
    __syncthreads();
    return *s_flag != 0;
}

__device__ __forceinline__ int round_half_up_pixel(float u) {
    const float c = fminf(fmaxf(u, -4.0f), 1.0e6f);
    const float f = floorf(c);
    return (int)f + ((c - f) >= 0.5f ? 1 : 0);
}
__device__ __forceinline__ unsigned lane_rank(unsigned long long m) {
    return __builtin_amdgcn_mbcnt_hi((unsigned)(m >> 32), __builtin_amdgcn_mbcnt_lo((unsigned)m, 0u));
}

typedef unsigned u32x4 __attribute__((ext_vector_type(4)));
__device__ __forceinline__ void st16(void *p, u32x4 v) { *reinterpret_cast<u32x4 *>(p) = v; }

struct FuseFrame {
    float inv[12];
    int ref;
    const FrameDev *frame;
};
struct FuseArgs {
    int W, H, nseeds, kf;
    int prevSlot;
    int rowScale;
    float fx, fy, cx, cy, fuseFar, fuseNear;
    const uint2 *tex; const float4 *fuseRec; uint8_t *fused;
    HotPk *hot; ColdRec *cold;
    long long *ctr;
    unsigned *blockSums, *blockUpd;
    unsigned *sbKeys;
    const unsigned *deal;
    unsigned *delOut;
    unsigned *delCount;
    DeferCtl *dc;
};
__host__ inline FuseArgs fuse_args(const SfDev &P, int slot, bool deferred, unsigned blkStride, bool dealt = false) {
    FuseArgs A;
    A.W = P.W; A.H = P.H; A.nseeds = P.nseeds; A.kf = P.kf; A.prevSlot = P.prevSlotAbs; A.rowScale = (254 << 16) / P.H;
    A.sbKeys = P.sbKeys; A.deal = dealt ? P.deal : nullptr;
    A.fx = P.fx; A.fy = P.fy; A.cx = P.cx; A.cy = P.cy; A.fuseFar = P.fuseFar; A.fuseNear = P.fuseNear;
    A.tex = P.tex + (size_t)slot * P.pxStride; A.fuseRec = P.fuseRec + (size_t)slot * P.nseeds * 3; A.fused = P.fused + (size_t)slot * P.flagStride;
    A.hot = P.map.hot; A.cold = P.map.cold; A.ctr = P.ctr;
    A.dc = P.dc;
    A.blockSums = P.blockSums; A.blockUpd = P.blockUpd + (size_t)(deferred ? P.kf : 0) * blkStride;
    A.delOut = deferred ? P.delList : P.delU;
    A.delCount = deferred ? &P.dc->delCnt[P.kf < DEFER_WIN ? P.kf : 0] : P.delUCount;
    return A;
}
__host__ inline FuseFrame fuse_frame(const FrameDev &F, const FrameDev *dev) {
    FuseFrame f;
    for (int c = 0; c < 4; c++) for (int r = 0; r < 3; r++) f.inv[3 * c + r] = F.invPose[4 * c + r];
    f.ref = F.ref; f.frame = dev;
    return f;
}

__device__ __forceinline__ unsigned spawn_word(unsigned fw) { return ~(fw | (fw >> 1)) & 0x01010101u; }
__device__ __forceinline__ unsigned spawn_count(const FuseArgs &P, unsigned lane, unsigned &excl) {
    const DeferCtl *dc = P.dc;
    const int fs = dc->flagStride;
    const uint8_t *fusedP = dc->fused + (size_t)P.prevSlot * fs;
    const int per = fs >> 6, nch = per >> 4;
    unsigned cnt = 0;
    const uint4 *fq = reinterpret_cast<const uint4 *>(fusedP + (size_t)lane * per);
    for (int c = 0; c < nch; c += 5) {
        uint4 b[5];
#pragma unroll
        for (int q = 0; q < 5; q++) b[q] = fq[min(c + q, nch - 1)];
#pragma unroll
        for (int q = 0; q < 5; q++)
            if (c + q < nch) cnt += (unsigned)(__popc(spawn_word(b[q].x)) + __popc(spawn_word(b[q].y)) + __popc(spawn_word(b[q].z)) + __popc(spawn_word(b[q].w)));
    }
    const unsigned incl = wave_incl_scan(cnt);
    excl = incl - cnt;
    return (unsigned)__builtin_amdgcn_readlane((int)incl, 63);
}
__device__ __forceinline__ void emit_records(const FuseArgs &P, long long E0, long long c0, int nj, unsigned lane, unsigned K, unsigned excl) {
    const DeferCtl *dc = P.dc;
    const int fs = dc->flagStride;
    const uint8_t *fusedP = dc->fused + (size_t)P.prevSlot * fs;
    const int per = fs >> 6, nch = per >> 4;
    const msl_surfel *cand = dc->cand + (size_t)P.prevSlot * P.nseeds;
#pragma unroll 1
    for (int j = 0; j < nj; j++) {
        const long long i = c0 + 64 * j + lane, kS = i - E0;
        const bool on = kS >= 0 && kS < (long long)K;
        const unsigned k = on ? (unsigned)kS : 0u;
        unsigned lo = 0, hi = 63, eLo = 0;
#pragma unroll
        for (int s = 0; s < 6; s++) {
            const unsigned mid = (lo + hi + 1) >> 1;
            const unsigned e = (unsigned)__builtin_amdgcn_ds_bpermute((int)(mid * 4u), (int)excl);
            if (e <= k) { lo = mid; eLo = e; } else hi = mid - 1;
        }
        unsigned r = k - eLo;
        int seed = -1;
        const uint4 *of = reinterpret_cast<const uint4 *>(fusedP + (size_t)lo * per);
        for (int c = 0; c < nch; c++) {
            const uint4 b = of[c];
            const unsigned w[4] = {spawn_word(b.x), spawn_word(b.y), spawn_word(b.z), spawn_word(b.w)};
#pragma unroll
            for (int q = 0; q < 4; q++) {
                const unsigned pc = (unsigned)__popc(w[q]);
                if (seed < 0) {
                    if (r < pc) {
                        unsigned m = w[q];
                        for (unsigned t = 0; t < r; t++) m &= m - 1;
                        seed = (int)lo * per + 16 * c + 4 * q + (__builtin_ctz(m) >> 3);
                    } else r -= pc;
                }
            }
        }
        if (on && seed >= 0) {
            if ((unsigned long long)i < dc->aux.cap) store_surfel(dc->aux.map, i, cand[seed]);
            else { long long code = 20; asm volatile("" : "+v"(code)); P.ctr[CTR_ERR] = code; }
        }
    }
    asm volatile("s_waitcnt vmcnt(0)" ::: "memory");
}

static_assert(SUB_ITEMS == 256 || SUB_ITEMS == 128 || SUB_ITEMS == 64, "k_fuse: four or two records per lane; k_compact lists a sub-block with one thread per slot");

}

#endif
```

### manhattanslam_amd/csrc/msl_sf_replay.hip

```cpp

#include "msl_sf_map_dev.h"

namespace {
__global__ __launch_bounds__(64) void k_defer_tail(SfDev P, FuseArgs A, int F, unsigned blkStride) {
    __builtin_amdgcn_s_setprio(3);
    const unsigned lane = threadIdx.x;
    if ((int)blockIdx.x < F) {
        const int f = (int)blockIdx.x;
        const long long E0 = f > 0 ? P.dc->ext[f - 1] : P.dc->ext[0], Kp = f > 0 ? P.dc->ext[f] - E0 : 0;
        const long long nblk = (E0 + SUB_ITEMS - 1) / SUB_ITEMS, x0 = E0 / SUB_ITEMS + 1, x1 = x0 + (Kp + SUB_ITEMS - 1) / SUB_ITEMS;
        const unsigned *bu = P.blockUpd + (size_t)f * blkStride;
        unsigned u = 0;
        for (long long b = lane; b < nblk; b += 64) u += bu[b];
        for (long long b = x0 + lane; b < x1; b += 64) u += bu[b];
        u = wave_incl_scan(u);
        if (lane == 63) {
            atomicAdd(reinterpret_cast<unsigned long long *>(&P.ctr[CTR_TOT_UPDATED]), (unsigned long long)u);
            if (f == F - 1) P.ctr[CTR_UPDATED] = u;
        }
        return;
    }
    const long long E0 = P.dc->ext[F - 1];
    const long long q = (long long)blockIdx.x - F, sb = E0 / SUB_ITEMS + q;
    if (sb * SUB_ITEMS >= E0 + P.nseeds) return;
    unsigned excl;
    const unsigned K = spawn_count(A, lane, excl);
    if (q == 0 && lane == 0) P.dc->ext[F] = E0 + (long long)K;
    if (K && sb * SUB_ITEMS < E0 + (long long)K) emit_records(A, E0, sb * SUB_ITEMS, SUB_ITEMS / 64, lane, K, excl);
}

constexpr int RP_SORT = 1024;
constexpr int RP_HASH = 2048;
constexpr unsigned RP_EMPTY = 0xFFFFFFFFu;
struct ReplayLds {
    unsigned v[RP_SORT + 4], d[RP_SORT];
    long long ext[DEFER_WIN + 1], runV[DEFER_WIN];
    unsigned runK0[DEFER_WIN], runCnt[DEFER_WIN];
    unsigned dcnt[DEFER_WIN];
    unsigned log[RP_HASH / 2];
    unsigned locK[RP_HASH], locV[RP_HASH], vposK[RP_HASH], vposV[RP_HASH];
};
__device__ __forceinline__ unsigned rp_hash(unsigned key) { return (key * 2654435761u) >> 21; }
static_assert(RP_HASH == 2048, "rp_hash yields 11 bits");

template <bool LDS>
__device__ __forceinline__ void replay_body(const SfDev &P, int F, ReplayLds &S) {
    const unsigned lane = threadIdx.x;
    DeferCtl *dc = P.dc;
    const long long n0 = S.ext[0];
    long long n = n0;
    unsigned nLocKeys = 0, nVposKeys = 0, logBase = 0;
    long long totK = 0, totD = 0, totNb = 0, lastK = 0, lastD = 0, lastNb = 0;
    auto loc_get = [&](unsigned p, unsigned &elem, unsigned &stampOut) -> bool {
        if constexpr (LDS) {
            for (unsigned s = rp_hash(p);; s = (s + 1) & (RP_HASH - 1)) {
                const unsigned k = S.locK[s];
                if (k == RP_EMPTY) return false;
                if (k == p) { const unsigned v = S.locV[s]; elem = (v & 0x3FFFFFFu) - 1u; stampOut = v >> 26; return true; }
            }
        } else {
            const unsigned long long v = ld_agent64(&P.loc64[p]);
            if (!v) return false;
            elem = (unsigned)v - 1u; stampOut = (unsigned)(v >> 32);
            return true;
        }
    };
    auto vpos_get = [&](unsigned id, unsigned &pos) -> bool {
        if constexpr (LDS) {
            for (unsigned s = rp_hash(id);; s = (s + 1) & (RP_HASH - 1)) {
                const unsigned k = S.vposK[s];
                if (k == RP_EMPTY) return false;
                if (k == id) { pos = S.vposV[s]; return true; }
            }
        } else {
            const unsigned v = ld_agent(&P.vposD[id]);
            if (!v) return false;
            pos = v - 1u;
            return true;
        }
    };
    auto put = [&](bool on, unsigned pos, unsigned elem, unsigned stampNo) {
        if constexpr (LDS) {
            if (on) {
                unsigned s = rp_hash(pos);
                for (;; s = (s + 1) & (RP_HASH - 1)) { const unsigned old = atomicCAS(&S.locK[s], RP_EMPTY, pos); if (old == RP_EMPTY || old == pos) break; }
                S.locV[s] = (elem + 1u) | (stampNo << 26);
                s = rp_hash(elem);
                for (;; s = (s + 1) & (RP_HASH - 1)) { const unsigned old = atomicCAS(&S.vposK[s], RP_EMPTY, elem); if (old == RP_EMPTY || old == elem) break; }
                S.vposV[s] = pos;
            }
        } else {
            if (on) { st_agent64(&P.loc64[pos], (unsigned long long)(elem + 1u) | ((unsigned long long)stampNo << 32)); st_agent(&P.vposD[elem], pos + 1u); }
            const unsigned long long m = __ballot(on);
            if (on) { const unsigned r = lane_rank(m); st_agent(&P.locKeys[nLocKeys + r], pos); st_agent(&P.vposKeys[nVposKeys + r], elem); }
            nLocKeys += (unsigned)__popcll(m); nVposKeys += (unsigned)__popcll(m);
        }
    };
    auto tables_sync = [&]() {
        if constexpr (LDS) __syncthreads();
        else { asm volatile("s_waitcnt vmcnt(0)" ::: "memory"); __syncthreads(); }
    };
    unsigned runMask = 0;
    auto vpos_of = [&](unsigned id) -> unsigned {
        unsigned pos;
        if (vpos_get(id, pos)) return pos;
        if ((long long)id < n0) return id;
        int g = 0;
        for (int q = 1; q < F; q++) if ((long long)id >= S.ext[q]) g = q;
        return (unsigned)(S.runV[g] + ((long long)id - S.ext[g] - (long long)S.runK0[g]));
    };
    auto run_of = [&](long long p, int upto, unsigned &elem) -> int {
        for (unsigned m = upto >= 31 ? runMask : (runMask & ((2u << upto) - 1u)); m;) {
            const int g = 31 - __builtin_clz(m);
            m &= ~(1u << g);
            const long long v0 = S.runV[g];
            if (p >= v0 && p < v0 + (long long)S.runCnt[g]) { elem = (unsigned)(S.ext[g] + (long long)S.runK0[g] + (p - v0)); return g; }
        }
        return -1;
    };
    auto loc_of = [&](long long p, int upto) -> unsigned {
        unsigned ee = 0, st = 0, er = 0;
        const bool have = loc_get((unsigned)p, ee, st);
        const int g = run_of(p, upto, er);
        if (have && (g < 0 || st > (unsigned)(g + 1))) return ee;
        return g >= 0 ? er : (unsigned)p;
    };
    for (int f = 0; f < F; f++) {
        const unsigned D = S.dcnt[f];
        const long long K = S.ext[f + 1] - S.ext[f];
        const unsigned stampNo = (unsigned)(f + 1);
        const bool inLds = D <= (unsigned)RP_SORT;
        lastK = K; lastD = D; lastNb = n; totK += K; totD += D; totNb += n;
        for (unsigned j0 = 0; j0 < D; j0 += 64) {
            const unsigned j = j0 + lane;
            if (j < D) {
                const unsigned vp = vpos_of(LDS ? S.log[logBase + j] : ld_agent(&P.delList[logBase + j]));
                if (inLds) S.v[j] = vp;
                else atomicOr(&P.bitmap[vp >> 5], 1u << (vp & 31u));
            }
        }
        if (inLds && lane < 4) S.v[D + lane] = 0xFFFFFFFFu;
        __syncthreads();
        if (inLds) {
            for (unsigned j0 = 0; j0 < D; j0 += 64) {
                const unsigned j = j0 + lane;
                const unsigned v = j < D ? S.v[j] : 0u;
                unsigned r = 0;
                for (unsigned q = 0; q < D; q += 4) {
                    const uint4 x = *reinterpret_cast<const uint4 *>(&S.v[q]);
                    r += (x.x < v ? 1u : 0u) + (x.y < v ? 1u : 0u) + (x.z < v ? 1u : 0u) + (x.w < v ? 1u : 0u);
                }
                if (j < D) S.d[r] = v;
            }
        } else {
            asm volatile("s_waitcnt vmcnt(0)" ::: "memory");
            const long long nw = (n + 31) >> 5;
            unsigned base = 0;
            for (long long w0 = 0; w0 < nw; w0 += 64) {
                const long long w = w0 + lane;
                unsigned bits = w < nw ? ld_agent(&P.bitmap[w]) : 0u;
                const unsigned c = (unsigned)__popc(bits);
                const unsigned incl = wave_incl_scan(c);
                unsigned o = base + incl - c;
                if (bits) st_agent(&P.bitmap[w], 0u);
                for (; bits; bits &= bits - 1) st_agent(&P.dBig[o++], (unsigned)(w * 32 + __builtin_ctz(bits)));
                base += (unsigned)__builtin_amdgcn_readlane((int)incl, 63);
            }
            asm volatile("s_waitcnt vmcnt(0)" ::: "memory");
        }
        __syncthreads();
        auto DL = [&](long long j) -> unsigned { return inLds ? S.d[j] : ld_agent(&P.dBig[j]); };
        const long long nPl = K < (long long)D ? K : (long long)D;
        for (long long k0 = 0; k0 < nPl; k0 += 64) {
            const long long k = k0 + lane;
            const bool on = k < nPl;
            put(on, on ? DL((long long)D - 1 - k) : 0u, (unsigned)(S.ext[f] + k), stampNo);
        }
        if (K > (long long)D) {
            if (lane == 0) { S.runV[f] = n; S.runK0[f] = D; S.runCnt[f] = (unsigned)(K - (long long)D); }
            runMask |= 1u << f;
            n += K - (long long)D;
        } else if ((long long)D > K) {
            const long long R = (long long)D - K, nFinal = n - R;
            tables_sync();
            auto lower = [&](long long x) -> long long {
                long long lo = 0, hi = R;
                while (lo < hi) { const long long mid = (lo + hi) >> 1; if ((long long)DL(mid) < x) lo = mid + 1; else hi = mid; }
                return lo;
            };
            const long long cntLow = lower(nFinal);
            for (long long a0 = 0; a0 < cntLow; a0 += 64) {
                const long long a = a0 + lane;
                const bool on = a < cntLow;
                long long p = nFinal + (on ? a : 0);
                bool chain = on;
                while (__ballot(chain)) {
                    if (chain) {
                        const long long lb = lower(p);
                        if (lb < R && (long long)DL(lb) == p) p = n - (R - lb);
                        else chain = false;
                    }
                }
                const unsigned e = on ? loc_of(p, f) : 0u;
                if constexpr (LDS) __syncthreads();
                put(on, on ? DL(a) : 0u, e, stampNo);
            }
            __syncthreads();
            if (runMask) {
                bool gone = false;
                if ((int)lane <= f && ((runMask >> lane) & 1u) && S.runV[lane] + (long long)S.runCnt[lane] > nFinal) {
                    S.runCnt[lane] = S.runV[lane] >= nFinal ? 0u : (unsigned)(nFinal - S.runV[lane]);
                    gone = S.runCnt[lane] == 0;
                }
                runMask &= ~(unsigned)__ballot(gone);
            }
            n = nFinal;
        }
        tables_sync();
        logBase += D;
    }
    const long long nF = n;
    unsigned nMoves = 0;
    auto add_move = [&](bool on, unsigned dst, unsigned src) {
        const unsigned long long m = __ballot(on);
        if (on) { const unsigned r = nMoves + lane_rank(m); P.moveDst[r] = dst; P.srcOf[r] = src; }
        nMoves += (unsigned)__popcll(m);
    };
    for (int g = 0; g < F; g++) {
        const unsigned cnt = ((runMask >> g) & 1u) ? S.runCnt[g] : 0u;
        for (unsigned q0 = 0; q0 < cnt; q0 += 64) {
            const unsigned q = q0 + lane;
            bool on = q < cnt;
            const long long p = S.runV[g] + q;
            const unsigned id = (unsigned)(S.ext[g] + (long long)S.runK0[g] + q);
            unsigned ee = 0, st = 0;
            if (on && loc_get((unsigned)p, ee, st) && st > (unsigned)(g + 1)) on = false;
            if (on && (long long)id == p) on = false;
            add_move(on, (unsigned)p, id);
        }
    }
    auto explicit_move = [&](bool on, unsigned p, unsigned id, unsigned st) {
        unsigned er = 0;
        if (on) { const int g = run_of((long long)p, F - 1, er); if (g >= 0 && (unsigned)(g + 1) > st) on = false; }
        if (on && (long long)p >= nF) on = false;
        if (on && id == p) on = false;
        add_move(on, p, id);
    };
    if constexpr (LDS) {
        for (unsigned s0 = 0; s0 < (unsigned)RP_HASH; s0 += 64) {
            const unsigned k = S.locK[s0 + lane], v = S.locV[s0 + lane];
            explicit_move(k != RP_EMPTY, k, (v & 0x3FFFFFFu) - 1u, v >> 26);
        }
    } else {
        for (unsigned j0 = 0; j0 < nLocKeys; j0 += 64) {
            const unsigned j = j0 + lane;
            bool on = j < nLocKeys;
            const unsigned p = on ? ld_agent(&P.locKeys[j]) : 0u;
            const unsigned long long v = on ? ld_agent64(&P.loc64[p]) : 0ull;
            on = on && v != 0ull;
            if (on) st_agent64(&P.loc64[p], 0ull);
            explicit_move(on, p, (unsigned)v - 1u, (unsigned)(v >> 32));
        }
        for (unsigned j0 = 0; j0 < nVposKeys; j0 += 64) { const unsigned j = j0 + lane; if (j < nVposKeys) st_agent(&P.vposD[ld_agent(&P.vposKeys[j])], 0u); }
    }
    if (lane < DEFER_WIN) dc->delCnt[lane] = 0;
    if (lane == 0) {
        dc->nMoves = nMoves;
        P.ctr[CTR_LIVE] = nF; P.ctr[CTR_NEW] = lastK; P.ctr[CTR_DELETED] = lastD; P.ctr[CTR_BEFORE] = lastNb; P.ctr[CTR_AFTER] = nF;
        P.ctr[CTR_TOT_NEW] += totK; P.ctr[CTR_TOT_DELETED] += totD; P.ctr[CTR_TOT_KF] += F; P.ctr[CTR_TOT_BEFORE] += totNb;
    }
}

__global__ __launch_bounds__(64) void k_replay(SfDev P, int F) {
    __shared__ __attribute__((aligned(16))) ReplayLds S;
    __builtin_amdgcn_s_setprio(3);
    const unsigned lane = threadIdx.x;
    DeferCtl *dc = P.dc;
    if ((int)lane <= F) S.ext[lane] = dc->ext[lane];
    if (lane < DEFER_WIN) { S.runCnt[lane] = 0; S.runV[lane] = 0; S.runK0[lane] = 0; }
    const unsigned dmine = (int)lane < F ? ld_agent(&dc->delCnt[lane]) : 0u;
    if (lane < DEFER_WIN) S.dcnt[lane] = dmine;
    const unsigned dsum = wave_incl_scan(dmine);
    const unsigned totalD = (unsigned)__builtin_amdgcn_readlane((int)dsum, 63);
    const bool useLds = totalD <= (unsigned)RP_HASH / 2 && P.cap < (1ull << 26) - 1;
    if (useLds) {
        for (unsigned j = lane; j < totalD; j += 64) S.log[j] = ld_agent(&P.delList[j]);
        for (unsigned s = lane; s < (unsigned)RP_HASH; s += 64) { S.locK[s] = RP_EMPTY; S.vposK[s] = RP_EMPTY; }
    }
    __syncthreads();
    if (useLds) replay_body<true>(P, F, S);
    else replay_body<false>(P, F, S);
}

__global__ __launch_bounds__(256) void k_gather(SfDev P) {
    const MapSoA &M = P.map;
    const unsigned nM = P.dc->nMoves;
    for (unsigned j = blockIdx.x * 256 + threadIdx.x; j < nM; j += gridDim.x * 256) {
        const unsigned s = P.srcOf[j];
        const HotPk h = M.hot[s];
        const ColdRec c = cold_load(M.cold + s);
        P.stageHot[j] = h; cold_store(P.stageCold + j, c);
        if (h.tl == HOT_WIDE) { P.stageUtl[2 * (size_t)j] = M.utlWide[2 * (size_t)s]; P.stageUtl[2 * (size_t)j + 1] = M.utlWide[2 * (size_t)s + 1]; }
        if (c.rgbf & COLD_WIDE) for (int q = 0; q < 3; q++) P.stageRgb[3 * (size_t)j + q] = M.rgbWide[3 * (size_t)s + q];
    }
}
__global__ __launch_bounds__(256) void k_scatter(SfDev P) {
    const MapSoA &M = P.map;
    const unsigned nM = P.dc->nMoves;
    for (unsigned j = blockIdx.x * 256 + threadIdx.x; j < nM; j += gridDim.x * 256) {
        const unsigned d = P.moveDst[j];
        const HotPk h = P.stageHot[j];
        const ColdRec c = cold_load(P.stageCold + j);
        M.hot[d] = h; cold_store(M.cold + d, c);
        if (h.tl == HOT_WIDE) { M.utlWide[2 * (size_t)d] = P.stageUtl[2 * (size_t)j]; M.utlWide[2 * (size_t)d + 1] = P.stageUtl[2 * (size_t)j + 1]; }
        if (c.rgbf & COLD_WIDE) for (int q = 0; q < 3; q++) M.rgbWide[3 * (size_t)d + q] = P.stageRgb[3 * (size_t)j + q];
    }
}
}

namespace msl {
namespace sf {
void map_launch_replay(KernelProfiler &prof, hipStream_t st, const SfDev &P, int F, unsigned blkStride) {
    const unsigned nFront = (unsigned)((P.nseeds + SUB_ITEMS - 1) / SUB_ITEMS) + 1u;
    hipLaunchKernelGGL(k_defer_tail, dim3((unsigned)F + nFront), dim3(64), 0, st, P, fuse_args(P, 0, true, blkStride), F, blkStride);
    MSL_SF_LAUNCH(prof, SK_COMPACT, st, k_replay, dim3(1), dim3(64), P, F);
    hipLaunchKernelGGL(k_gather, dim3(128), dim3(256), 0, st, P);
    hipLaunchKernelGGL(k_scatter, dim3(128), dim3(256), 0, st, P);
}
}
}
```

### manhattanslam_amd/csrc/msl_sf_store.hip

```cpp

#include "msl_sf_handle.h"

#include <cmath>
#include <fstream>
#include <vector>

namespace msl {
namespace sf {

namespace {

constexpr size_t HOT_W = sizeof(HotPk) / 4, COLD_W = sizeof(ColdRec) / 4;
constexpr size_t ST_HOT = 0, ST_COLD = ST_HOT + HOT_W, ST_RGB = ST_COLD + COLD_W, ST_UTL = ST_RGB + 3, MAP_WORDS = ST_UTL + 2;
constexpr size_t RP_LOC64 = 0, RP_STAGE_COLD = RP_LOC64 + 2, RP_STAGE_HOT = RP_STAGE_COLD + COLD_W, RP_MOVE_DST = RP_STAGE_HOT + HOT_W, RP_VPOS_D = RP_MOVE_DST + 1,
                 RP_LOC_KEYS = RP_VPOS_D + 1, RP_VPOS_KEYS = RP_LOC_KEYS + 1, RP_DBIG = RP_VPOS_KEYS + 1, RP_STAGE_RGB = RP_DBIG + 1, RP_STAGE_UTL = RP_STAGE_RGB + 3,
                 RP_BITMAP = RP_STAGE_UTL + 2, RP_WORDS = RP_BITMAP;
constexpr size_t rp_bitmap_words(size_t c) { return c / 32 + 64; }
static_assert(ST_HOT == 0 && ST_COLD == 4 && ST_RGB == 12 && ST_UTL == 15 && MAP_WORDS == 17, "layout of map.store");
static_assert(RP_LOC64 == 0 && RP_STAGE_COLD == 2 && RP_STAGE_HOT == 10 && RP_MOVE_DST == 14 && RP_VPOS_D == 15 && RP_LOC_KEYS == 16 && RP_VPOS_KEYS == 17 &&
              RP_DBIG == 18 && RP_STAGE_RGB == 19 && RP_STAGE_UTL == 22 && RP_BITMAP == 24 && RP_WORDS == 24, "layout of map.rp");
constexpr size_t round_cap(size_t n) { return (n + 4095) & ~(size_t)4095; }

void set_map_ptrs(msl_sf *h, size_t c) {
    MapSoA &M = h->dev.map;
    float *store = (float *)h->map.store.p;
    M.hot = reinterpret_cast<HotPk *>(store + ST_HOT * c);
    M.cold = reinterpret_cast<ColdRec *>(store + ST_COLD * c);
    M.rgbWide = reinterpret_cast<int *>(store + ST_RGB * c);
    M.utlWide = reinterpret_cast<int *>(store + ST_UTL * c);
    M.wideFlag = h->dev.ctr + CTR_WIDE;
    SfDev &D = h->dev;
    D.cap = c;
    D.blockSums = (unsigned *)h->map.blockSums.p; D.blockUpd = (unsigned *)h->map.blockUpd.p; D.delList = (unsigned *)h->map.delList.p; D.srcOf = (unsigned *)h->map.srcOf.p;
    D.sbKeys = D.blockSums + h->blkStride; D.deal = D.blockSums + 2 * h->blkStride; D.dealG = 0;
    unsigned *r = (unsigned *)h->map.rp.p;
    D.loc64 = reinterpret_cast<unsigned long long *>(r + RP_LOC64 * c);
    D.stageCold = reinterpret_cast<ColdRec *>(r + RP_STAGE_COLD * c);
    D.stageHot = reinterpret_cast<HotPk *>(r + RP_STAGE_HOT * c);
    D.moveDst = r + RP_MOVE_DST * c; D.vposD = r + RP_VPOS_D * c; D.locKeys = r + RP_LOC_KEYS * c; D.vposKeys = r + RP_VPOS_KEYS * c; D.dBig = r + RP_DBIG * c;
    D.stageRgb = reinterpret_cast<int *>(r + RP_STAGE_RGB * c); D.stageUtl = reinterpret_cast<int *>(r + RP_STAGE_UTL * c);
    D.bitmap = r + RP_BITMAP * c;
}

struct StorePlane { size_t word, bytes; long long wide; };
constexpr StorePlane kStorePlanes[4] = {{ST_HOT, sizeof(HotPk), 0}, {ST_COLD, sizeof(ColdRec), 0}, {ST_RGB, sizeof(int) * 3, 1}, {ST_UTL, sizeof(int) * 2, 2}};
constexpr long long ALL_PLANES = 3;
int copy_store(void *dst, size_t dstCap, const void *src, size_t srcCap, size_t n, long long wide, const hipStream_t *async) {
    for (const StorePlane &pl : kStorePlanes) {
        if (pl.wide && !(wide & pl.wide)) continue;
        float *d = (float *)dst + pl.word * dstCap;
        const float *s = (const float *)src + pl.word * srcCap;
        if (async) MSL_HIP_TRY(hipMemcpyAsync(d, s, pl.bytes * n, hipMemcpyDeviceToDevice, *async));
        else MSL_HIP_TRY(hipMemcpy(d, s, pl.bytes * n, hipMemcpyDeviceToDevice));
    }
    return MSL_OK;
}
size_t snap_cap(const msl_sf *h) { return h->d_snapStore.cap / (sizeof(float) * MAP_WORDS); }

void drop_live_snapshots(msl_sf *h) {
    for (int i = 0; i < msl_sf::NSNAP; i++) h->snapLive[i] = false;
}

void consume_snapshots(msl_sf *h, size_t nseeds) {
    for (int i = 0; i < msl_sf::NSNAP; i++)
        if (h->snapBusy[i] && hipEventQuery(h->snapEv[i]) == hipSuccess) {
            h->snapBusy[i] = false;
            const long long *sn = (const long long *)h->h_snap.p + (size_t)i * msl_sf::SNAPW;
            if (h->snapLive[i]) {
                const size_t cand = (size_t)sn[CTR_LIVE] + (size_t)(h->kfEnq - h->snapKf[i]) * nseeds;
                if (cand < h->liveBound) h->liveBound = cand;
                if (h->snapKf[i] >= h->liveKnownKf) { h->liveKnown = (size_t)sn[CTR_LIVE]; h->liveKnownKf = h->snapKf[i]; }
            }
            if (h->snapKf[i] > h->churnAt) {
                if (h->churnNew >= 0 && sn[CTR_TOT_KF] > h->churnKf)
                    h->churn = (double)((sn[CTR_TOT_NEW] - h->churnNew) + (sn[CTR_TOT_DELETED] - h->churnDel)) / (double)(sn[CTR_TOT_KF] - h->churnKf);
                h->churnNew = sn[CTR_TOT_NEW]; h->churnDel = sn[CTR_TOT_DELETED]; h->churnKf = sn[CTR_TOT_KF]; h->churnAt = h->snapKf[i];
            }
        }
}

}

int write_ctl(msl_sf *h) {
    DeferCtl dc;
    memset(&dc, 0, sizeof(dc));
    const SfDev &D = h->dev;
    dc.flagStride = D.flagStride; dc.candOk = D.candOk; dc.fused = D.fused; dc.cand = D.cand;
    dc.aux.map = D.map; dc.aux.cap = D.cap; dc.aux.delU = D.delU; dc.aux.delUCount = D.delUCount; dc.aux.delList = D.delList;
    MSL_HIP_TRY(hipMemcpy(D.dc, &dc, sizeof(dc), hipMemcpyHostToDevice));
    return MSL_OK;
}

int map_realloc(msl_sf *h, size_t cap, size_t keep) {
    cap = round_cap(cap);
    const size_t bst = cap / SUB_ITEMS + 8200;
    const size_t rpWords = RP_WORDS * cap + rp_bitmap_words(cap);
    msl_sf::MapBufs m;
    MSL_HIP_TRY(grow_all(h->mapStream, {{m.store, sizeof(float) * MAP_WORDS * cap},
                                        {m.blockSums, sizeof(unsigned) * 3 * bst},
                                        {m.blockUpd, sizeof(unsigned) * DEFER_WIN * bst},
                                        {m.delList, sizeof(unsigned) * cap}, {m.srcOf, sizeof(unsigned) * cap}, {m.rp, sizeof(unsigned) * rpWords}}));
    unsigned *nbs = (unsigned *)m.blockSums.p, *nrp = (unsigned *)m.rp.p;
    MSL_HIP_TRY(hipMemset(nbs, 0, sizeof(unsigned) * bst));
    MSL_HIP_TRY(hipMemset(nbs + bst, 0xFF, sizeof(unsigned) * bst));
    MSL_HIP_TRY(hipMemset(m.blockUpd.p, 0, sizeof(unsigned) * DEFER_WIN * bst));
    MSL_HIP_TRY(hipMemset(nrp + RP_LOC64 * cap, 0, sizeof(unsigned long long) * cap));
    MSL_HIP_TRY(hipMemset(nrp + RP_VPOS_D * cap, 0, sizeof(unsigned) * cap));
    MSL_HIP_TRY(hipMemset(nrp + RP_BITMAP * cap, 0, sizeof(unsigned) * rp_bitmap_words(cap)));
    if (keep && h->map.store.p) {
        int rc = sync_all(h);
        if (rc != MSL_OK) return rc;
        rc = copy_store(m.store.p, cap, h->map.store.p, h->dev.cap, keep, ALL_PLANES, nullptr);
        if (rc != MSL_OK) return rc;
    }
    h->map = std::move(m);
    h->blkStride = bst;
    h->dealG = 0;
    set_map_ptrs(h, cap);
    return write_ctl(h);
}

int read_ctr(msl_sf *h) {
    if (h->ownStreams && h->copyStream) MSL_HIP_TRY(hipStreamSynchronize(h->copyStream));
    MSL_HIP_TRY(hipStreamSynchronize(h->preStream));
    MSL_HIP_TRY(hipMemcpyAsync(h->h_ctr.p, h->dev.ctr, sizeof(long long) * CTR_COUNT, hipMemcpyDeviceToHost, h->mapStream));
    MSL_HIP_TRY(hipStreamSynchronize(h->mapStream));
    h->prof.drain();
    consume_snapshots(h, (size_t)h->dev.nseeds);
    h->liveBound = live_count(h);
    h->liveKnown = h->liveBound; h->liveKnownKf = h->kfEnq;
    for (int i = 0; i < msl_sf::NSNAP; i++) h->snapBusy[i] = false;
    return MSL_OK;
}

int check_err(msl_sf *h) {
    const long long e = host_ctr(h, CTR_ERR);
    if (e) {
        (void)hipMemsetAsync(h->dev.ctr + CTR_ERR, 0, sizeof(long long), h->mapStream);
        if (e == 20) set_error("resident surfel map capacity exceeded (reserve more with msl_sf_map_reserve)");
        else set_error("surfel pipeline device-side bound exceeded (code %lld)", e);
        return MSL_ERR_OVERFLOW;
    }
    return MSL_OK;
}

int reserve_map(msl_sf *h, int n) {
    const SfDev &D = h->dev;
    h->mirrorValid = false;
    const size_t need = (size_t)n * (size_t)D.nseeds;
    consume_snapshots(h, (size_t)D.nseeds);
    if (h->liveBound + need > D.cap) {
        int rc = settle(h);
        if (rc != MSL_OK) return rc;
        if (h->liveBound + need > D.cap) {
            rc = map_realloc(h, 2 * h->liveBound + 2 * need + 65536, h->liveBound);
            if (rc != MSL_OK) return rc;
        }
    }
    h->liveBound += need;
    h->kfEnq += (unsigned long long)n;
    return MSL_OK;
}

void map_replaced(msl_sf *h, size_t n) {
    h->liveBound = n; h->liveKnown = n; h->liveKnownKf = h->kfEnq; h->classicNext = true;
    drop_live_snapshots(h);
}

int aos_in(msl_sf *h, const msl_surfel *host, size_t n, bool atEnd) {
    const hipStream_t s = h->mapStream;
    MSL_HIP_TRY(h->d_aos.grow(sizeof(msl_surfel) * n, s));
    MSL_HIP_TRY(hipMemcpyAsync(h->d_aos.p, host, sizeof(msl_surfel) * n, hipMemcpyHostToDevice, s));
    map_launch_aos_to_soa(h->prof, s, h->dev, (const msl_surfel *)h->d_aos.p, (long long)n, atEnd);
    return MSL_OK;
}

int aos_out(msl_sf *h, size_t n, const MapSelect *sel, msl_surfel *host, const AosRun *runs, size_t nRuns) {
    const hipStream_t s = h->mapStream;
    MSL_HIP_TRY(h->d_aos.grow(sizeof(msl_surfel) * n, s));
    msl_surfel *aos = (msl_surfel *)h->d_aos.p;
    if (sel) map_launch_select_write(s, h->dev, sel->mode, sel->arg, aos, sel->mark ? 1 : 0);
    else map_launch_soa_to_aos(h->prof, s, h->dev, aos, (long long)n);
    for (size_t r = 0; r < nRuns; r++)
        MSL_HIP_TRY(hipMemcpyAsync(host + runs[r].i0, aos + runs[r].i0, sizeof(msl_surfel) * (runs[r].i1 - runs[r].i0), hipMemcpyDeviceToHost, s));
    return MSL_OK;
}

namespace {

int map_select(msl_sf *h, const MapSelect &sel, msl_surfel *out, size_t cap, size_t *n_out, const char *what) {
    if (!h || !n_out) { set_error("%s: invalid argument", what); return MSL_ERR_INVALID; }
    if (sel.mark) { h->mirrorValid = false; h->classicNext = true; }
    MSL_HIP_TRY(hipSetDevice(h->device));
    int rc = settle(h);
    if (rc != MSL_OK) return rc;
    *n_out = 0;
    if (live_count(h) == 0) return MSL_OK;
    const hipStream_t s = h->mapStream;
    map_launch_select_count(s, h->dev, sel.mode, sel.arg);
    rc = read_ctr(h);
    if (rc != MSL_OK) return rc;
    const size_t m = (size_t)host_ctr(h, CTR_SELECTED);
    *n_out = m;
    (void)hipMemsetAsync(h->dev.ctr + CTR_SELECTED, 0, sizeof(long long), s);
    if (m > cap || (m && !out)) { set_error("%s: %zu surfels selected, capacity %zu", what, m, cap); return MSL_ERR_CAPACITY; }
    if (m == 0) return MSL_OK;
    const AosRun all{0, m};
    rc = aos_out(h, m, &sel, out, &all, 1);
    if (rc != MSL_OK) return rc;
    MSL_HIP_TRY(hipStreamSynchronize(s));
    return MSL_OK;
}

}

}
}

using namespace msl;
using namespace msl::sf;

extern "C" {

int msl_sf_map_reserve(msl_sf *h, size_t capacity) noexcept {
    try {
    if (!h) return MSL_ERR_INVALID;
    MSL_HIP_TRY(hipSetDevice(h->device));
    if (capacity <= h->dev.cap) return MSL_OK;
    int rc = read_ctr(h);
    if (rc != MSL_OK) return rc;
    return map_realloc(h, capacity, live_count(h));
    } MSL_ABI_CATCH_INT
}

int msl_sf_map_upload(msl_sf *h, const msl_surfel *host, size_t n) noexcept {
    try {
    if (!h || (n && !host)) return MSL_ERR_INVALID;
    h->mirrorValid = false;
    MSL_HIP_TRY(hipSetDevice(h->device));
    int rc = sync_all(h);
    if (rc != MSL_OK) return rc;
    if (n + (size_t)h->dev.nseeds > h->dev.cap) {
        rc = map_realloc(h, n + n / 4 + 4 * (size_t)h->dev.nseeds, 0);
        if (rc != MSL_OK) return rc;
    }
    hipStream_t s = h->mapStream;
    MSL_HIP_TRY(hipMemsetAsync(h->dev.ctr + CTR_WIDE, 0, sizeof(long long), s));
    if (n) {
        rc = aos_in(h, host, n, false);
        if (rc != MSL_OK) return rc;
    }
    map_launch_set_ctr(s, h->dev, (long long)n, -1);
    MSL_HIP_TRY(hipStreamSynchronize(s));
    map_replaced(h, n);
    return MSL_OK;
    } MSL_ABI_CATCH_INT
}

int msl_sf_map_snapshot(msl_sf *h) noexcept {
    try {
    if (!h) return MSL_ERR_INVALID;
    MSL_HIP_TRY(hipSetDevice(h->device));
    int rc = settle(h);
    if (rc != MSL_OK) return rc;
    const size_t n = live_count(h);
    const long long wide = host_ctr(h, CTR_WIDE);
    h->snapValid = false;
    MSL_HIP_TRY(h->d_snapStore.grow(sizeof(float) * MAP_WORDS * round_cap(n), h->mapStream));
    if (n) {
        rc = copy_store(h->d_snapStore.p, snap_cap(h), h->map.store.p, h->dev.cap, n, wide, nullptr);
        if (rc != MSL_OK) return rc;
    }
    h->snapN = n; h->snapValid = true; h->snapWide = wide;
    return MSL_OK;
    } MSL_ABI_CATCH_INT
}

int msl_sf_map_restore(msl_sf *h) noexcept {
    try {
    if (!h || !h->snapValid) { set_error("msl_sf_map_restore: no snapshot"); return MSL_ERR_INVALID; }
    h->mirrorValid = false;
    MSL_HIP_TRY(hipSetDevice(h->device));
    const size_t n = h->snapN;
    int rc;
    if (n + (size_t)h->dev.nseeds > h->dev.cap) {
        rc = read_ctr(h);
        if (rc != MSL_OK) return rc;
        rc = map_realloc(h, n + n / 4 + 4 * (size_t)h->dev.nseeds, 0);
        if (rc != MSL_OK) return rc;
    }
    const hipStream_t s = h->mapStream;
    if (n) {
        rc = copy_store(h->map.store.p, h->dev.cap, h->d_snapStore.p, snap_cap(h), n, h->snapWide, &s);
        if (rc != MSL_OK) return rc;
    }
    map_launch_set_ctr(s, h->dev, (long long)n, (int)h->snapWide);
    MSL_HIP_TRY(hipGetLastError());
    map_replaced(h, n);
    return MSL_OK;
    } MSL_ABI_CATCH_INT
}

int msl_sf_map_size(msl_sf *h, size_t *n_out) noexcept {
    try {
    if (!h || !n_out) return MSL_ERR_INVALID;
    MSL_HIP_TRY(hipSetDevice(h->device));
    int rc = read_ctr(h);
    if (rc != MSL_OK) return rc;
    *n_out = live_count(h);
    return check_err(h);
    } MSL_ABI_CATCH_INT
}

int msl_sf_map_download(msl_sf *h, msl_surfel *host, size_t cap, size_t *n_out) noexcept {
    try {
    if (!h || !n_out) return MSL_ERR_INVALID;
    MSL_HIP_TRY(hipSetDevice(h->device));
    int rc = read_ctr(h);
    if (rc != MSL_OK) return rc;
    const size_t n = live_count(h);
    *n_out = n;
    if (n > cap || (n && !host)) { set_error("msl_sf_map_download: capacity %zu < map size %zu", cap, n); return MSL_ERR_CAPACITY; }
    if (n) {
        const AosRun all{0, n};
        rc = aos_out(h, n, nullptr, host, &all, 1);
        if (rc != MSL_OK) return rc;
        MSL_HIP_TRY(hipStreamSynchronize(h->mapStream));
    }
    return check_err(h);
    } MSL_ABI_CATCH_INT
}

int msl_sf_map_detach(msl_sf *h, int pose_index, msl_surfel *out, size_t cap, size_t *n_out) noexcept { try {
    return map_select(h, {0, pose_index, true}, out, cap, n_out, "msl_sf_map_detach"); } MSL_ABI_CATCH_INT }
int msl_sf_map_export(msl_sf *h, int min_update_times, msl_surfel *out, size_t cap, size_t *n_out) noexcept { try {
    return map_select(h, {1, min_update_times, false}, out, cap, n_out, "msl_sf_map_export"); } MSL_ABI_CATCH_INT }
int msl_sf_export_ply(msl_sf *h, int min_update_times, const msl_surfel *inactive, size_t n_inactive, const char *path) noexcept {
    try {
    if (!h || !path || (n_inactive && !inactive)) { set_error("msl_sf_export_ply: invalid argument"); return MSL_ERR_INVALID; }
    size_t n = 0;
    int rc = msl_sf_map_export(h, min_update_times, nullptr, 0, &n);
    if (rc != MSL_OK && rc != MSL_ERR_CAPACITY) return rc;
    std::vector<msl_surfel> pts(n + n_inactive);
    if (n) { rc = msl_sf_map_export(h, min_update_times, pts.data(), n, &n); if (rc != MSL_OK) return rc; }
    for (size_t i = 0; i < n_inactive; i++) pts[n + i] = inactive[i];
    size_t count = 0;
    for (const msl_surfel &e : pts) count += std::isnan(e.px) ? 0 : 1;
    std::ofstream os(path, std::ios::out);
    if (os.fail()) { set_error("msl_sf_export_ply: cannot open %s", path); return MSL_ERR_INVALID; }
    os << "ply\nformat ascii 1.0\nelement vertex " << count << "\n";
    for (const char *p : {"x", "y", "z", "nx", "ny", "nz"}) os << "property float " << p << "\n";
    for (const char *p : {"red", "green", "blue", "alpha"}) os << "property uchar " << p << "\n";
    for (const char *p : {"quality", "radius"}) os << "property float " << p << "\n";
    os << "element camera 1\n";
    for (const char *p : {"view_px", "view_py", "view_pz", "x_axisx", "x_axisy", "x_axisz", "y_axisx", "y_axisy", "y_axisz", "z_axisx", "z_axisy", "z_axisz",
                          "focal", "scalex", "scaley", "centerx", "centery"})
        os << "property float " << p << "\n";
    os << "property int viewportx\nproperty int viewporty\nproperty float k1\nproperty float k2\nend_header\n";
    for (const msl_surfel &e : pts) {
        if (std::isnan(e.px)) continue;
        os << e.px << " " << e.py << " " << e.pz << " " << e.nx << " " << e.ny << " " << e.nz << " " << (unsigned)(uint8_t)e.r << " " << (unsigned)(uint8_t)e.g << " "
           << (unsigned)(uint8_t)e.b << " 1 " << e.weight << " " << e.size * 1000 << "\n";
    }
    os << "0 0 0 1 0 0 0 1 0 0 0 1 0 0 0 0 0 " << (int)count << " 1 0 0\n";
    return os.fail() ? MSL_ERR_INVALID : MSL_OK;
    } MSL_ABI_CATCH_INT
}

int msl_sf_map_append(msl_sf *h, const msl_surfel *surfels, size_t n) noexcept {
    try {
    if (!h || (n && !surfels)) { set_error("msl_sf_map_append: invalid argument"); return MSL_ERR_INVALID; }
    h->mirrorValid = false;
    MSL_HIP_TRY(hipSetDevice(h->device));
    int rc = read_ctr(h);
    if (rc != MSL_OK) return rc;
    if (n == 0) return MSL_OK;
    const size_t cur = live_count(h);
    if (cur + n + (size_t)h->dev.nseeds > h->dev.cap) {
        rc = map_realloc(h, cur + n + (cur + n) / 4 + 4 * (size_t)h->dev.nseeds, cur);
        if (rc != MSL_OK) return rc;
    }
    rc = aos_in(h, surfels, n, true);
    if (rc != MSL_OK) return rc;
    map_launch_add_ctr(h->mapStream, h->dev, (long long)n);
    MSL_HIP_TRY(hipStreamSynchronize(h->mapStream));
    map_replaced(h, cur + n);
    return MSL_OK;
    } MSL_ABI_CATCH_INT
}

int msl_sf_last_counters(msl_sf *h, int64_t counters[5]) noexcept {
    try {
    if (!h || !counters) return MSL_ERR_INVALID;
    MSL_HIP_TRY(hipSetDevice(h->device));
    int rc = read_ctr(h);
    if (rc != MSL_OK) return rc;
    const SfCtr order[5] = {CTR_BEFORE, CTR_NEW, CTR_DELETED, CTR_UPDATED, CTR_LIVE};
    for (int i = 0; i < 5; i++) counters[i] = host_ctr(h, order[i]);
    return check_err(h);
    } MSL_ABI_CATCH_INT
}

}
```

### manhattanslam_amd/csrc/msl_surfel.hip

```cpp

#include "msl_sf_handle.h"

#include <algorithm>
#include <cstdlib>
#include <memory>
#include <vector>

namespace msl {
namespace sf {

int sync_all(msl_sf *h) {
    if (h->ownStreams && h->copyStream) MSL_HIP_TRY(hipStreamSynchronize(h->copyStream));
    MSL_HIP_TRY(hipStreamSynchronize(h->preStream));
    MSL_HIP_TRY(hipStreamSynchronize(h->mapStream));
    return MSL_OK;
}

void release_staged_images(msl_sf *h) {
    msl_sf::Slots &S = h->slot;
    S.gray = msl_sf::ImageSlots(); S.depth = msl_sf::ImageSlots(); S.member = msl_sf::ImageSlots();
    h->stagedSet = -1;
}

int alloc_slots(msl_sf *h, int maxBatch) {
    release_staged_images(h);
    h->slot = msl_sf::Slots();
    msl_sf::Slots &S = h->slot;
    SfDev &D = h->dev;
    const size_t slots = 2 * (size_t)maxBatch, ns = D.nseeds, npx = D.pxStride, fs = D.flagStride;
    MSL_HIP_TRY(grow_all(h->mapStream, {{S.frames, sizeof(FrameDev) * slots}, {S.seeds, sizeof(msl_seed) * ns * slots}, {S.seedsTmp, sizeof(msl_seed) * ns * slots},
                                        {S.cand, sizeof(msl_surfel) * ns * slots}, {S.candOk, fs * slots}, {S.fused, fs * slots},
                                        {S.tex, sizeof(uint2) * npx * slots}, {S.fuseRec, sizeof(float4) * 3 * ns * slots},
                                        {S.index, sizeof(unsigned short) * npx * slots}, {S.amap, sizeof(unsigned short) * npx * slots}, {S.tmin, sizeof(unsigned) * ns * slots},
                                        {S.arec, sizeof(AssignRec) * (ns * slots + 2)},
                                        {S.pxInv, sizeof(float) * npx * slots}, {S.wl, sizeof(unsigned) * npx * slots}, {S.wlCount, sizeof(unsigned) * slots},
                                        {S.chunkAbort, sizeof(int) * 32 * slots}, {S.changed, sizeof(int) * 8 * slots}}));
    MSL_HIP_TRY(S.hFrames.grow(sizeof(FrameDev) * slots, h->mapStream));
    MSL_HIP_TRY(hipMemset(S.tex.p, 0, S.tex.cap));
    MSL_HIP_TRY(hipMemset(S.fuseRec.p, 0, S.fuseRec.cap));
    MSL_HIP_TRY(hipMemset(S.wlCount.p, 0, S.wlCount.cap));
    MSL_HIP_TRY(hipMemset(S.arec.p, 0, S.arec.cap));
    MSL_HIP_TRY(hipMemset(S.seeds.p, 0, S.seeds.cap));
    MSL_HIP_TRY(hipMemset(S.index.p, 0, S.index.cap));
    MSL_HIP_TRY(hipMemset(S.fused.p, 1, S.fused.cap));
    MSL_HIP_TRY(hipMemset(S.candOk.p, 0, S.candOk.cap));
    D.frames = (FrameDev *)S.frames.p; D.seeds = (msl_seed *)S.seeds.p; D.seedsTmp = (msl_seed *)S.seedsTmp.p; D.cand = (msl_surfel *)S.cand.p;
    D.candOk = (uint8_t *)S.candOk.p; D.fused = (uint8_t *)S.fused.p; D.tex = (uint2 *)S.tex.p; D.fuseRec = (float4 *)S.fuseRec.p;
    D.index = (unsigned short *)S.index.p; D.amap = (unsigned short *)S.amap.p; D.tmin = (unsigned *)S.tmin.p; D.chunkAbort = (int *)S.chunkAbort.p; D.changed = (int *)S.changed.p;
    D.arec = (AssignRec *)S.arec.p + 1; D.pxInv = (float *)S.pxInv.p; D.wl = (unsigned *)S.wl.p; D.wlCount = (unsigned *)S.wlCount.p;
    { const int rc = write_ctl(h); if (rc != MSL_OK) return rc; }
    h->maxBatch = maxBatch;
    h->lastSlot = 0;
    for (msl_sf::SlotSet &t : h->sets) t.preValid = t.mapValid = t.copyValid = false;
    return MSL_OK;
}

namespace {

int check_images(const msl_sf *h, int n, const int32_t *refs, const float *poses, BatchImages &I) {
    const size_t W = (size_t)h->dev.W, H = (size_t)h->dev.H;
    ImageArg &g = I.gray, &d = I.depth, &r = I.depth16, &m = I.member;
    if (n < 1 || n > h->maxBatch) { set_error("msl_sf: batch of %d keyframes exceeds the batch capacity %d", n, h->maxBatch); return MSL_ERR_INVALID; }
    if (I.d16()) {
        if (r.row < W * 2 || (r.row & 1) || (r.frame & 1) || ((uintptr_t)r.p & 1)) { set_error("msl_sf: bad 16-bit depth pointer or strides"); return MSL_ERR_INVALID; }
        d.row = W * 4; d.frame = d.row * H;
    }
    if (!g.p || (!d.p && !I.d16()) || !m.p || !poses || !refs || g.row < W || d.row < W * 4 || m.row < ((W + 1) / 2) * 4 || (d.row & 3) || (m.row & 3)) {
        set_error("msl_sf: bad image pointers or strides");
        return MSL_ERR_INVALID;
    }
    if (g.row * H >= (1ull << 32) || d.row * H >= (1ull << 32) || m.row * ((H + 1) / 2) >= (1ull << 32)) {
        set_error("msl_sf: image rows span 4 GB or more");
        return MSL_ERR_INVALID;
    }
    g.bytes = g.row * (H - 1) + W; d.bytes = d.row * (H - 1) + W * 4;
    m.bytes = m.row * ((H + 1) / 2 - 1) + ((W + 1) / 2) * 4;
    r.bytes = I.d16() ? r.row * (H - 1) + W * 2 : 0;
    return MSL_OK;
}

int copy_frames(uint8_t *dst, size_t dstStride, int n, const void *src, size_t frameStride, size_t bytes, hipStream_t st) {
    if (frameStride == bytes && dstStride == bytes) {
        MSL_HIP_TRY(hipMemcpyAsync(dst, src, bytes * (size_t)n, hipMemcpyHostToDevice, st));
        return MSL_OK;
    }
    for (int f = 0; f < n; f++) MSL_HIP_TRY(hipMemcpyAsync(dst + f * dstStride, (const uint8_t *)src + f * frameStride, bytes, hipMemcpyHostToDevice, st));
    return MSL_OK;
}

struct FrameSrc { const uint8_t *gray, *depth, *member; size_t grayStep, depthStep, memberStep; };

int stage_images(msl_sf *h, int set, int n, const BatchImages &I, FrameSrc &src) {
    msl_sf::Slots &S = h->slot;
    msl_sf::SlotSet &T = h->sets[set];
    const ImageArg &g = I.gray, &d = I.depth, &r = I.depth16, &m = I.member;
    const int W = h->dev.W, H = h->dev.H;
    const size_t slot0 = (size_t)set * (size_t)h->maxBatch, slots = 2 * (size_t)h->maxBatch;
    const hipStream_t sp = h->preStream, sm = h->mapStream;
    if (I.mem != MSL_MEM_HOST) {
        h->stagedSet = -1;
        src = {(const uint8_t *)g.p, (const uint8_t *)d.p, (const uint8_t *)m.p, g.frame, d.frame, m.frame};
        if (!I.d16()) return MSL_OK;
        if (d.bytes > S.depth.stride) {
            const int rc = sync_all(h);
            if (rc != MSL_OK) return rc;
            release_staged_images(h);
            MSL_HIP_TRY(S.depth.buf.grow(d.bytes * slots, sm));
            S.depth.stride = d.bytes;
        }
        sp_launch_depth_u16(sp, r.p, r.row, r.frame, (float *)S.depth.at(slot0), S.depth.stride / 4, W, H, n, I.depthFactor);
        src.depth = S.depth.at(slot0); src.depthStep = S.depth.stride;
        return MSL_OK;
    }
    if (g.bytes > S.gray.stride || d.bytes > S.depth.stride || m.bytes > S.member.stride) {
        const int rc = sync_all(h);
        if (rc != MSL_OK) return rc;
        release_staged_images(h);
        MSL_HIP_TRY(grow_all(sm, {{S.gray.buf, g.bytes * slots}, {S.depth.buf, d.bytes * slots}, {S.member.buf, m.bytes * slots}}));
        S.gray.stride = g.bytes; S.depth.stride = d.bytes; S.member.stride = m.bytes;
    }
    if (r.bytes > S.depth16.stride) {
        const int rc = sync_all(h);
        if (rc != MSL_OK) return rc;
        S.depth16.stride = 0;
        MSL_HIP_TRY(S.depth16.buf.grow(r.bytes * slots, sm));
        S.depth16.stride = r.bytes;
    }
    const hipStream_t sc = (h->ownStreams && h->copyStream) ? h->copyStream : sp;
    if (sc != sp && T.preValid) MSL_HIP_TRY(hipStreamWaitEvent(sc, T.pre, 0));
    h->prof.begin(SK_COPY, sc);
    int rc = copy_frames(S.gray.at(slot0), S.gray.stride, n, g.p, g.frame, g.bytes, sc);
    if (rc == MSL_OK) rc = I.d16() ? copy_frames(S.depth16.at(slot0), S.depth16.stride, n, r.p, r.frame, r.bytes, sc)
                                   : copy_frames(S.depth.at(slot0), S.depth.stride, n, d.p, d.frame, d.bytes, sc);
    if (rc == MSL_OK) rc = copy_frames(S.member.at(slot0), S.member.stride, m.frame == 0 ? 1 : n, m.p, m.frame, m.bytes, sc);
    if (rc != MSL_OK) return rc;
    if (I.d16())
        sp_launch_depth_u16(sc, S.depth16.at(slot0), r.row, S.depth16.stride, (float *)S.depth.at(slot0), S.depth.stride / 4, W, H, n, I.depthFactor);
    h->prof.end(sc);
    MSL_HIP_TRY(hipEventRecord(T.h2d, sc));
    if (sc != sp) MSL_HIP_TRY(hipStreamWaitEvent(sp, T.h2d, 0));
    h->stagedSet = set; h->stagedGs = g.row;
    src = {S.gray.at(slot0), S.depth.at(slot0), S.member.at(slot0), S.gray.stride, S.depth.stride, m.frame == 0 ? 0 : S.member.stride};
    return MSL_OK;
}

int fill_frames(msl_sf *h, int set, int n, const FrameSrc &src, const int32_t *refs, const float *poses) {
    msl_sf::SlotSet &T = h->sets[set];
    const size_t slot0 = (size_t)set * (size_t)h->maxBatch;
    if (T.copyValid) MSL_HIP_TRY(hipEventSynchronize(T.copy));
    FrameDev *hf = (FrameDev *)h->slot.hFrames.p + slot0;
    for (int f = 0; f < n; f++) {
        FrameDev &F = hf[f];
        F.gray = src.gray + f * src.grayStep;
        F.depth = (const float *)(src.depth + f * src.depthStep);
        F.member = (const int32_t *)(src.member + f * src.memberStep);
        memcpy(F.pose, poses + 16 * f, sizeof(float) * 16);
        inverse4<float>(F.pose, F.invPose);
        F.ref = refs[f]; F._pad = 0;
    }
    MSL_HIP_TRY(hipMemcpyAsync((FrameDev *)h->slot.frames.p + slot0, hf, sizeof(FrameDev) * n, hipMemcpyHostToDevice, h->preStream));
    MSL_HIP_TRY(hipEventRecord(T.copy, h->preStream));
    T.copyValid = true;
    return MSL_OK;
}

SfDev slot_view(const SfDev &D, int slot0) {
    SfDev P = D;
    P.frames = D.frames + slot0; P.seeds = D.seeds + (size_t)slot0 * D.nseeds; P.seedsTmp = D.seedsTmp + (size_t)slot0 * D.nseeds;
    P.cand = D.cand + (size_t)slot0 * D.nseeds; P.candOk = D.candOk + (size_t)slot0 * D.flagStride; P.fused = D.fused + (size_t)slot0 * D.flagStride;
    P.tex = D.tex + (size_t)slot0 * D.pxStride; P.fuseRec = D.fuseRec + (size_t)slot0 * D.nseeds * 3;
    P.index = D.index + (size_t)slot0 * D.pxStride; P.amap = D.amap + (size_t)slot0 * D.pxStride; P.tmin = D.tmin + (size_t)slot0 * D.nseeds;
    P.arec = D.arec + (size_t)slot0 * D.nseeds; P.pxInv = D.pxInv + (size_t)slot0 * D.pxStride; P.wl = D.wl + (size_t)slot0 * D.pxStride; P.wlCount = D.wlCount + slot0;
    P.chunkAbort = D.chunkAbort + slot0 * 32; P.changed = D.changed + slot0 * 8;
    return P;
}

struct SfPolicy {
    int dealEvery;
    bool dealOff;
    bool deferOff, deferForce;
};
const SfPolicy &sf_policy() {
    static const SfPolicy p = [] {
        const char *every = getenv("MSL_SF_DEAL_EVERY"), *deal = getenv("MSL_SF_DEAL"), *defer = getenv("MSL_SF_DEFER");
        return SfPolicy{every ? std::max(1, atoi(every)) : 4, deal && !strcmp(deal, "0"), defer && !strcmp(defer, "0"), defer && !strcmp(defer, "1")};
    }();
    return p;
}
constexpr double CHURN_MAX = 96.0;
constexpr int DEAL_MAX_GRID = (4 << 20) / SUB_ITEMS;

struct FuseGrid { int nSubGrid, nSubHint; bool dealOn; };
FuseGrid fuse_grid(const msl_sf *h, bool compact) {
    const SfDev &D = h->dev;
    const size_t boundLive = compact ? h->liveBound : D.cap;
    const size_t known = std::min(h->liveKnown, boundLive);
    const size_t subWant = (std::min(known + 2 * (size_t)D.nseeds, boundLive) + SUB_ITEMS - 1) / SUB_ITEMS;
    FuseGrid g;
    g.nSubGrid = (int)std::max<size_t>(8, std::min((subWant + 63) & ~(size_t)63, (size_t)D.cap / SUB_ITEMS));
    g.nSubHint = (int)(known / SUB_ITEMS);
    g.dealOn = !sf_policy().dealOff && (g.nSubGrid & 7) == 0 && (size_t)g.nSubGrid <= h->blkStride && g.nSubGrid <= DEAL_MAX_GRID;
    return g;
}

int launch_map_chain(msl_sf *h, SfDev &P, int set, int n, bool compact) {
    const SfPolicy &pol = sf_policy();
    const hipStream_t sp = h->preStream, sm = h->mapStream;
    const int slot0 = set * h->maxBatch;
    const FrameDev *hf = (const FrameDev *)h->slot.hFrames.p + slot0;
    const FuseGrid g = fuse_grid(h, compact);
    const bool churny = !pol.deferForce && (h->churn > CHURN_MAX || sp != sm);
    auto classic = [&](int f) {
        P.kf = 0;
        map_launch_fuse(h->prof, sm, P, f, hf[f], g.nSubGrid, g.nSubHint, false, g.dealOn && h->dealG == g.nSubGrid, (unsigned)h->blkStride);
        P.dealG = g.dealOn && compact && (f % pol.dealEvery == 0 || h->dealG != g.nSubGrid) ? g.nSubGrid : 0;
        map_launch_compact(h->prof, sm, P, f, compact);
        if (P.dealG) h->dealG = g.nSubGrid;
        h->kfClassic++;
    };
    int f = 0;
    const int fProbe = n / 2;
    if (!compact || pol.deferOff || churny || n < 2) {
        for (; f < n; f++) { classic(f); if (f == fProbe) map_launch_empty_pair(h->prof, sm); }
    } else {
        if (h->classicNext) { classic(0); f = 1; if (fProbe == 0) map_launch_empty_pair(h->prof, sm); }
        while (f < n) {
            const int w = std::min(DEFER_WIN, n - f);
            for (int q = 0; q < w; q++) {
                P.kf = q; P.prevSlotAbs = slot0 + f + q - 1;
                map_launch_fuse(h->prof, sm, P, f + q, hf[f + q], g.nSubGrid, g.nSubHint, true, g.dealOn && h->dealG == g.nSubGrid, (unsigned)h->blkStride);
                if (f + q == fProbe) map_launch_empty_pair(h->prof, sm);
            }
            P.kf = w; P.prevSlotAbs = slot0 + f + w - 1;
            map_launch_replay(h->prof, sm, P, w, (unsigned)h->blkStride);
            h->kfDeferred += (unsigned long long)w;
            if (g.dealOn) { P.dealG = g.nSubGrid; map_launch_deal(sm, P); h->dealG = g.nSubGrid; }
            f += w;
        }
    }
    if (compact) h->classicNext = false;
    if (sp != sm) { MSL_HIP_TRY(hipEventRecord(h->sets[set].map, sm)); h->sets[set].mapValid = true; }
    if (compact && h->h_snap.p) {
        const int i = h->snapNext;
        if (!h->snapBusy[i]) {
            MSL_HIP_TRY(hipMemcpyAsync((long long *)h->h_snap.p + (size_t)i * msl_sf::SNAPW, h->dev.ctr, sizeof(long long) * msl_sf::SNAPW, hipMemcpyDeviceToHost, sm));
            MSL_HIP_TRY(hipEventRecord(h->snapEv[i], sm));
            h->snapKf[i] = h->kfEnq; h->snapBusy[i] = true; h->snapLive[i] = true; h->snapNext = (i + 1) % msl_sf::NSNAP;
        }
    }
    MSL_HIP_TRY(hipGetLastError());
    h->lastSlot = slot0 + n - 1;
    h->batchNo++;
    return MSL_OK;
}

}

int run_batch(msl_sf *h, int n, const int32_t *refs, const float *poses, BatchImages I, bool compact) {
    int rc = check_images(h, n, refs, poses, I);
    if (rc != MSL_OK) return rc;
    if (compact) {
        rc = reserve_map(h, n);
        if (rc != MSL_OK) return rc;
    }
    SfDev &D = h->dev;
    const int set = (int)(h->batchNo & 1);
    msl_sf::SlotSet &T = h->sets[set];
    const hipStream_t sp = h->preStream, sm = h->mapStream;
    if (T.mapValid && sp != sm) MSL_HIP_TRY(hipStreamWaitEvent(sp, T.map, 0));
    D.gstride = I.gray.row; D.gbytes = I.gray.bytes; D.dstride = I.depth.row / 4; D.mstride = I.member.row / 4;
    D.gsB = (unsigned)I.gray.row; D.dsB = (unsigned)I.depth.row; D.msB = (unsigned)I.member.row;
    FrameSrc src;
    rc = stage_images(h, set, n, I, src);
    if (rc != MSL_OK) return rc;
    rc = fill_frames(h, set, n, src, refs, poses);
    if (rc != MSL_OK) return rc;
    SfDev P = slot_view(D, set * h->maxBatch);
    sp_launch_stage(h->prof, sp, P, n, h->propLds);
    if (sp != sm) {
        MSL_HIP_TRY(hipEventRecord(T.pre, sp));
        T.preValid = true;
        MSL_HIP_TRY(hipStreamWaitEvent(sm, T.pre, 0));
    }
    return launch_map_chain(h, P, set, n, compact);
}

}
}

using namespace msl;
using namespace msl::sf;

extern "C" {

msl_sf *msl_sf_create(int width, int height, float fx, float fy, float cx, float cy, float fuseFar, float fuseNear, int device) noexcept {
    try {
    if (width < 16 || height < 16 || fx == 0 || fy == 0 || (width / SP) * (height / SP) >= IDX_PLANE || (long long)width * height >= (1ll << 31)) {
        set_error("msl_sf_create: width/height must be >= 16 with fewer than 65534 superpixels, fx and fy non-zero");
        return nullptr;
    }
    if (bind_device(device) != MSL_OK) return nullptr;
    std::unique_ptr<msl_sf, void (*)(msl_sf *)> guard(new msl_sf, [](msl_sf *p) { msl_sf_destroy(p); });
    msl_sf *h = guard.get();
    h->device = device;
    SfDev &D = h->dev;
    D.W = width; D.H = height; D.spW = width / SP; D.spH = height / SP; D.nseeds = D.spW * D.spH; D.npx = width * height;
    D.pxStride = (D.npx + 63) & ~63;
    D.flagStride = 64 * ((((D.nseeds + 63) / 64) + 15) & ~15);
    D.fx = fx; D.fy = fy; D.cx = cx; D.cy = cy; D.fuseFar = fuseFar; D.fuseNear = fuseNear;
    bool ok = true;
    {
        int lo = 0, hi = 0;
        ok = ok && hipDeviceGetStreamPriorityRange(&lo, &hi) == hipSuccess;
        ok = ok && hipStreamCreateWithPriority(&h->preStream, hipStreamNonBlocking, lo) == hipSuccess;
        ok = ok && hipStreamCreateWithPriority(&h->mapStream, hipStreamNonBlocking, hi) == hipSuccess;
        ok = ok && hipStreamCreateWithFlags(&h->copyStream, hipStreamNonBlocking) == hipSuccess;
    }
    for (msl_sf::SlotSet &t : h->sets)
        for (hipEvent_t *e : {&t.pre, &t.map, &t.copy, &t.h2d}) ok = ok && hipEventCreateWithFlags(e, hipEventDisableTiming) == hipSuccess;
    const hipStream_t sm = h->mapStream;
    ok = ok && h->d_ctr.grow(sizeof(long long) * 32, sm) == hipSuccess;
    ok = ok && hipMemset(h->d_ctr.p, 0, sizeof(long long) * 32) == hipSuccess;
    ok = ok && h->h_ctr.grow(sizeof(long long) * 16, sm) == hipSuccess;
    ok = ok && h->h_snap.grow(sizeof(long long) * msl_sf::NSNAP * msl_sf::SNAPW, sm) == hipSuccess;
    for (int i = 0; i < msl_sf::NSNAP && ok; i++) ok = hipEventCreateWithFlags(&h->snapEv[i], hipEventDisableTiming) == hipSuccess;
    ok = ok && h->d_new.grow(sizeof(msl_surfel) * D.nseeds, sm) == hipSuccess;
    ok = ok && h->d_tickets.grow(sizeof(unsigned) * 8, sm) == hipSuccess && hipMemset(h->d_tickets.p, 0, sizeof(unsigned) * 8) == hipSuccess;
    ok = ok && h->d_delU.grow(sizeof(unsigned) * LIST_D, sm) == hipSuccess;
    ok = ok && h->d_dc.grow(sizeof(DeferCtl), sm) == hipSuccess && hipMemset(h->d_dc.p, 0, sizeof(DeferCtl)) == hipSuccess;
    {
        std::vector<float> tab((size_t)width + 1 + height + 1);
        for (int u = 0; u <= width; u++) tab[u] = ((float)u - cx) / fx;
        for (int v = 0; v <= height; v++) tab[(size_t)width + 1 + v] = ((float)v - cy) / fy;
        ok = ok && h->d_projTab.grow(sizeof(float) * tab.size(), sm) == hipSuccess;
        ok = ok && hipMemcpy(h->d_projTab.p, tab.data(), sizeof(float) * tab.size(), hipMemcpyHostToDevice) == hipSuccess;
        D.colX = (const float *)h->d_projTab.p; D.rowY = D.colX + width + 1;
    }
    if (ok) h->propLds = sp_init_attributes(D.nseeds);
    if (!ok) { set_error("msl_sf_create: HIP allocation failed"); return nullptr; }
    memset(h->h_ctr.p, 0, sizeof(long long) * 16);
    D.ctr = (long long *)h->d_ctr.p; D.newSurfels = (msl_surfel *)h->d_new.p; D.tickets = (unsigned *)h->d_tickets.p; D.delU = (unsigned *)h->d_delU.p;
    D.delUCount = D.tickets + 4; D.dc = (DeferCtl *)h->d_dc.p; D.kf = 0; D.prevSlotAbs = 0;
    h->prof.nk = MSL_SF_NKERNELS;
    if (alloc_slots(h, 1) != MSL_OK || map_realloc(h, 1 << 16, 0) != MSL_OK) return nullptr;
    return guard.release();
    } MSL_ABI_CATCH_PTR
}

void msl_sf_destroy(msl_sf *h) noexcept {
    try {
    if (!h) return;
    (void)hipSetDevice(h->device);
    if (h->copyStream) (void)hipStreamSynchronize(h->copyStream);
    if (h->preStream) (void)hipStreamSynchronize(h->preStream);
    if (h->mapStream) (void)hipStreamSynchronize(h->mapStream);
    h->prof.destroy();
    for (int i = 0; i < msl_sf::NSNAP; i++) if (h->snapEv[i]) (void)hipEventDestroy(h->snapEv[i]);
    for (const msl_sf::SlotSet &t : h->sets)
        for (hipEvent_t e : {t.pre, t.map, t.copy, t.h2d}) if (e) (void)hipEventDestroy(e);
    const hipStream_t streams[3] = {h->copyStream, h->ownStreams ? h->preStream : nullptr, h->ownStreams ? h->mapStream : nullptr};
    delete h;
    for (hipStream_t st : streams) if (st) (void)hipStreamDestroy(st);
    } MSL_ABI_CATCH_VOID
}

int msl_sf_staged_gray(msl_sf *h, const uint8_t **gray_dev, size_t *row_stride, size_t *frame_stride, void **uploaded_event) noexcept {
    try {
    if (!h || !gray_dev || !row_stride || !frame_stride || !uploaded_event) return MSL_ERR_INVALID;
    if (h->stagedSet < 0) { set_error("msl_sf_staged_gray: the last batch had no host images"); return MSL_ERR_INVALID; }
    *gray_dev = h->slot.gray.at((size_t)h->stagedSet * (size_t)h->maxBatch);
    *row_stride = h->stagedGs; *frame_stride = h->slot.gray.stride; *uploaded_event = (void *)h->sets[h->stagedSet].h2d;
    return MSL_OK;
    } MSL_ABI_CATCH_INT
}

int msl_sf_set_stream(msl_sf *h, void *hip_stream) noexcept {
    try {
    if (!h) return MSL_ERR_INVALID;
    MSL_HIP_TRY(hipSetDevice(h->device));
    int rc = sync_all(h);
    if (rc != MSL_OK) return rc;
    if (h->ownStreams) { (void)hipStreamDestroy(h->preStream); (void)hipStreamDestroy(h->mapStream); }
    h->preStream = h->mapStream = (hipStream_t)hip_stream; h->ownStreams = false;
    return MSL_OK;
    } MSL_ABI_CATCH_INT
}

int msl_sf_set_batch_capacity(msl_sf *h, int max_frames) noexcept {
    try {
    if (!h || max_frames < 1 || max_frames > 4096) { set_error("msl_sf_set_batch_capacity: invalid argument"); return MSL_ERR_INVALID; }
    MSL_HIP_TRY(hipSetDevice(h->device));
    int rc = sync_all(h);
    if (rc != MSL_OK) return rc;
    if (max_frames == h->maxBatch) return MSL_OK;
    return alloc_slots(h, max_frames);
    } MSL_ABI_CATCH_INT
}

int msl_sf_sync(msl_sf *h) noexcept {
    try {
    if (!h) return MSL_ERR_INVALID;
    MSL_HIP_TRY(hipSetDevice(h->device));
    return settle(h);
    } MSL_ABI_CATCH_INT
}

int msl_sf_fuse_resident_batch(msl_sf *h, int n_frames, const int32_t *refs, const uint8_t *gray, size_t gray_stride,
                               size_t gray_frame_stride, const float *depth, size_t depth_stride, size_t depth_frame_stride,
                               const int32_t *member, size_t member_stride, size_t member_frame_stride, msl_mem img_mem,
                               const float *poses_colmajor) noexcept {
    try {
    if (!h) { set_error("msl_sf_fuse_resident_batch: NULL handle"); return MSL_ERR_INVALID; }
    MSL_HIP_TRY(hipSetDevice(h->device));
    return run_batch(h, n_frames, refs, poses_colmajor, {{gray, gray_stride, gray_frame_stride}, {depth, depth_stride, depth_frame_stride}, {},
                                                         {member, member_stride, member_frame_stride}, img_mem}, true);
    } MSL_ABI_CATCH_INT
}

int msl_sf_fuse_resident_batch_d16(msl_sf *h, int n_frames, const int32_t *refs, const uint8_t *gray, size_t gray_stride, size_t gray_frame_stride,
                                   const uint16_t *depth16, size_t depth16_stride, size_t depth16_frame_stride, float depth_factor,
                                   const int32_t *member, size_t member_stride, size_t member_frame_stride, msl_mem img_mem,
                                   const float *poses_colmajor) noexcept {
    try {
    if (!h) { set_error("msl_sf_fuse_resident_batch_d16: NULL handle"); return MSL_ERR_INVALID; }
    if (!depth16) { set_error("msl_sf_fuse_resident_batch_d16: NULL depth"); return MSL_ERR_INVALID; }
    MSL_HIP_TRY(hipSetDevice(h->device));
    return run_batch(h, n_frames, refs, poses_colmajor, {{gray, gray_stride, gray_frame_stride}, {}, {depth16, depth16_stride, depth16_frame_stride},
                                                         {member, member_stride, member_frame_stride}, img_mem, depth_factor}, true);
    } MSL_ABI_CATCH_INT
}

int msl_sf_fuse_resident(msl_sf *h, int referenceFrameIndex, const uint8_t *gray, size_t gray_stride, const float *depth,
                         size_t depth_stride, const int32_t *member, size_t member_stride, msl_mem img_mem,
                         const float pose_colmajor[16]) noexcept {
    try {
    if (!h) { set_error("msl_sf_fuse_resident: NULL handle"); return MSL_ERR_INVALID; }
    MSL_HIP_TRY(hipSetDevice(h->device));
    const int32_t ref = referenceFrameIndex;
    return run_batch(h, 1, &ref, pose_colmajor, {{gray, gray_stride}, {depth, depth_stride}, {}, {member, member_stride}, img_mem}, true);
    } MSL_ABI_CATCH_INT
}

int msl_sf_profile_enable(msl_sf *h, int on) noexcept {
    try {
    if (!h) return MSL_ERR_INVALID;
    MSL_HIP_TRY(hipSetDevice(h->device));
    int rc = sync_all(h);
    if (rc != MSL_OK) return rc;
    h->prof.drain();
    h->prof.set_mode(on);
    return MSL_OK;
    } MSL_ABI_CATCH_INT
}
int msl_sf_profile_stride(msl_sf *h, int stride) noexcept {
    try {
    if (!h || stride < 1) return MSL_ERR_INVALID;
    h->prof.stride = stride;
    return MSL_OK;
    } MSL_ABI_CATCH_INT
}
int msl_sf_profile_read(msl_sf *h, float *ms, int32_t *launches) noexcept {
    try {
    if (!h) return MSL_ERR_INVALID;
    MSL_HIP_TRY(hipSetDevice(h->device));
    int rc = sync_all(h);
    if (rc != MSL_OK) return rc;
    h->prof.drain();
    for (int i = 0; i < MSL_SF_NKERNELS; i++) { if (ms) ms[i] = h->prof.ms[i]; if (launches) launches[i] = h->prof.launches[i]; }
    return MSL_OK;
    } MSL_ABI_CATCH_INT
}

}
```

### manhattanslam_amd/surfel.py

```python
import ctypes as C

import numpy as np

from ._lib import (MSL_MEM_DEVICE, MSL_MEM_HOST, MSL_SF_NKERNELS, SEED_DTYPE, SURFEL_DTYPE, MslError, check, lib, ptr)


def _pose16(pose):
    pose = np.asarray(pose, np.float32)
    if pose.shape == (4, 4):
        pose = pose.T.reshape(16)
    assert pose.shape == (16,)
    return np.ascontiguousarray(pose)


class SurfelFusion:

    def __init__(self, width, height, fx, fy, cx, cy, fuseFar, fuseNear, device=0):
        self._h = lib.msl_sf_create(int(width), int(height), float(fx), float(fy), float(cx), float(cy), float(fuseFar),
                                    float(fuseNear), int(device))
        if not self._h:
            raise MslError("msl_sf_create failed: " + lib.msl_last_error().decode())
        self.width, self.height = int(width), int(height)
        self.nseeds = (self.width // 8) * (self.height // 8)

    def close(self):
        if getattr(self, "_h", None):
            lib.msl_sf_destroy(self._h)
            self._h = None

    __del__ = close

    def fuseInitializeMap(self, referenceFrameIndex, inputImage, inputDepth, inputPlaneMembershipImg, pose, localSurfels, local_unchanged=False):
        g = inputImage if inputImage.strides[1] == 1 else np.ascontiguousarray(inputImage)
        d = inputDepth if inputDepth.strides[1] == 4 else np.ascontiguousarray(inputDepth)
        m = inputPlaneMembershipImg if inputPlaneMembershipImg.strides[1] == 4 else np.ascontiguousarray(inputPlaneMembershipImg)
        assert g.dtype == np.uint8 and d.dtype == np.float32 and m.dtype == np.int32
        assert localSurfels.dtype == SURFEL_DTYPE and localSurfels.flags.c_contiguous
        new = np.zeros(self.nseeds, SURFEL_DTYPE)
        n_new = C.c_size_t(0)
        p = _pose16(pose)
        check(lib.msl_sf_fuse_ex(self._h, int(referenceFrameIndex), ptr(g), g.strides[0], ptr(d), d.strides[0], ptr(m), m.strides[0],
                                 ptr(p), ptr(localSurfels) if len(localSurfels) else None, len(localSurfels), ptr(new), len(new),
                                 C.byref(n_new), 1 if local_unchanged else 0), "msl_sf_fuse_ex")
        return new[:n_new.value].copy()

    def map_reserve(self, cap):
        check(lib.msl_sf_map_reserve(self._h, int(cap)), "msl_sf_map_reserve")

    def map_upload(self, surfels):
        surfels = np.ascontiguousarray(surfels, SURFEL_DTYPE)
        check(lib.msl_sf_map_upload(self._h, ptr(surfels) if len(surfels) else None, len(surfels)), "msl_sf_map_upload")

    def map_snapshot(self):
        check(lib.msl_sf_map_snapshot(self._h), "msl_sf_map_snapshot")

    def map_restore(self):
        check(lib.msl_sf_map_restore(self._h), "msl_sf_map_restore")

    def map_size(self):
        n = C.c_size_t(0)
        check(lib.msl_sf_map_size(self._h, C.byref(n)), "msl_sf_map_size")
        return n.value

    def map_download(self):
        n = self.map_size()
        out = np.zeros(n, SURFEL_DTYPE)
        got = C.c_size_t(0)
        check(lib.msl_sf_map_download(self._h, ptr(out) if n else None, n, C.byref(got)), "msl_sf_map_download")
        return out[:got.value]

    def map_detach(self, pose_index):
        return self._select(lib.msl_sf_map_detach, pose_index, "msl_sf_map_detach")

    def map_export(self, min_update_times=5):
        return self._select(lib.msl_sf_map_export, min_update_times, "msl_sf_map_export")

    def _select(self, fn, arg, what):
        n = C.c_size_t(0)
        out = np.zeros(0, SURFEL_DTYPE)
        rc = fn(self._h, int(arg), None, 0, C.byref(n))
        if rc == 0:
            return out
        if rc != -4:
            check(rc, what)
        out = np.zeros(n.value, SURFEL_DTYPE)
        check(fn(self._h, int(arg), ptr(out), len(out), C.byref(n)), what)
        return out[:n.value]

    def export_ply(self, path, min_update_times=5, inactive=None):
        ina = np.zeros(0, SURFEL_DTYPE) if inactive is None else np.ascontiguousarray(inactive, SURFEL_DTYPE)
        check(lib.msl_sf_export_ply(self._h, int(min_update_times), ptr(ina) if len(ina) else None, len(ina), str(path).encode()), "msl_sf_export_ply")

    def map_append(self, surfels):
        surfels = np.ascontiguousarray(surfels, SURFEL_DTYPE)
        check(lib.msl_sf_map_append(self._h, ptr(surfels) if len(surfels) else None, len(surfels)), "msl_sf_map_append")

    def fuse_resident(self, referenceFrameIndex, gray, depth, member, pose, device=False, strides=None):
        if strides is None:
            strides = (gray.stride(0) if device else gray.strides[0], (depth.stride(0) * 4) if device else depth.strides[0],
                       (member.stride(0) * 4) if device else member.strides[0])
        p = _pose16(pose)
        check(lib.msl_sf_fuse_resident(self._h, int(referenceFrameIndex), ptr(gray), strides[0], ptr(depth), strides[1], ptr(member),
                                       strides[2], MSL_MEM_DEVICE if device else MSL_MEM_HOST, ptr(p)), "msl_sf_fuse_resident")

    def set_batch_capacity(self, max_frames):
        check(lib.msl_sf_set_batch_capacity(self._h, int(max_frames)), "msl_sf_set_batch_capacity")

    def fuse_resident_batch(self, refs, grays, depths, members, poses, device=False, member_shared=False, frame_step=1, member_frame_step=None,
                            depth_factor=None):
        n = len(refs)
        k = int(frame_step)
        km = k if member_frame_step is None else int(member_frame_step)
        refs = np.ascontiguousarray(refs, np.int32)
        poses = np.ascontiguousarray(np.stack([_pose16(p) for p in poses]), np.float32)
        w, h = self.width, self.height
        mw, mh = (w + 1) // 2, (h + 1) // 2
        if depth_factor is not None:
            check(lib.msl_sf_fuse_resident_batch_d16(self._h, n, ptr(refs), ptr(grays), w, k * w * h, ptr(depths), 2 * w, 2 * k * w * h, float(depth_factor),
                                                     ptr(members), 4 * mw, 0 if member_shared else 4 * km * mw * mh,
                                                     MSL_MEM_DEVICE if device else MSL_MEM_HOST, ptr(poses)), "msl_sf_fuse_resident_batch_d16")
            return
        check(lib.msl_sf_fuse_resident_batch(self._h, n, ptr(refs), ptr(grays), w, k * w * h, ptr(depths), 4 * w, 4 * k * w * h, ptr(members),
                                             4 * mw, 0 if member_shared else 4 * km * mw * mh,
                                             MSL_MEM_DEVICE if device else MSL_MEM_HOST, ptr(poses)), "msl_sf_fuse_resident_batch")

    def staged_gray(self):
        p, rs, fs, ev = C.c_void_p(), C.c_size_t(), C.c_size_t(), C.c_void_p()
        check(lib.msl_sf_staged_gray(self._h, C.byref(p), C.byref(rs), C.byref(fs), C.byref(ev)), "msl_sf_staged_gray")
        return p.value, rs.value, fs.value, ev.value

    def counters(self):
        c = np.zeros(5, np.int64)
        check(lib.msl_sf_last_counters(self._h, ptr(c)), "msl_sf_last_counters")
        return dict(zip(("n_live_before", "n_new", "n_deleted", "n_updated", "n_live_after"), (int(v) for v in c)))

    def sync(self):
        check(lib.msl_sf_sync(self._h), "msl_sf_sync")

    def set_stream(self, hip_stream):
        check(lib.msl_sf_set_stream(self._h, C.c_void_p(hip_stream)))

    def debug_seeds(self):
        out = np.zeros(self.nseeds, SEED_DTYPE)
        check(lib.msl_sf_debug_seeds(self._h, ptr(out)))
        return out

    def debug_ctr(self):
        out = np.zeros(16, np.int64)
        check(lib.msl_sf_debug_ctr(self._h, ptr(out)))
        return out

    def debug_scratch(self, n_words, which=0, offset=0):
        out = np.zeros(n_words, np.uint32)
        check(lib.msl_sf_debug_scratch(self._h, int(which), int(offset), ptr(out), n_words))
        return out

    def debug_event_overhead(self, grid=1, n=200):
        us = C.c_float(0)
        check(lib.msl_sf_debug_event_overhead(self._h, int(grid), int(n), C.byref(us)))
        return float(us.value)

    def debug_index(self):
        out = np.zeros((self.height, self.width), np.int32)
        check(lib.msl_sf_debug_index(self._h, ptr(out)))
        return out

    def profile_stride(self, stride=1):
        check(lib.msl_sf_profile_stride(self._h, int(stride)))

    def profile_enable(self, mode=-1):
        check(lib.msl_sf_profile_enable(self._h, int(mode)))

    @staticmethod
    def kernel_names():
        return [lib.msl_sf_kernel_name(k).decode() for k in range(MSL_SF_NKERNELS)]

    def profile_read(self):
        ms = np.zeros(MSL_SF_NKERNELS, np.float32)
        cnt = np.zeros(MSL_SF_NKERNELS, np.int32)
        check(lib.msl_sf_profile_read(self._h, ptr(ms), ptr(cnt)))
        return {lib.msl_sf_kernel_name(k).decode(): (float(ms[k]), int(cnt[k])) for k in range(MSL_SF_NKERNELS)}


class SurfelMap(SurfelFusion):

    def fuseMap(self, image, depth, planeMembershipImg, pose, referenceIndex, device=False):
        self.fuse_resident(referenceIndex, image, depth, planeMembershipImg, pose, device=device)
```

Before: 26910.

## Skip surfel sub-blocks whose cached bounding box lies outside the view frustum

New measurement: 26330. -2.2%, worse.

```diff
diff --git a/manhattanslam_amd/csrc/msl_sf.h b/manhattanslam_amd/csrc/msl_sf.h
--- a/manhattanslam_amd/csrc/msl_sf.h
+++ b/manhattanslam_amd/csrc/msl_sf.h
@@ -1,6 +1,7 @@
 #pragma once
 
 #include "msl_common.h"
+#include "msl_sf_bound.h"
 
 #include <hip/hip_ext.h>
 
@@ -43,7 +44,8 @@
     CTR_SELECTED = 7,
     CTR_TOT_NEW = 8, CTR_TOT_DELETED = 9, CTR_TOT_UPDATED = 10, CTR_TOT_KF = 11, CTR_TOT_BEFORE = 12,
     CTR_WIDE = 13,
-    CTR_COUNT = 16
+    CTR_COUNT = 16,
+    CTR_SB_TOT = 32, SB_TOT_SLOTS = 128, CTR_ALLOC = CTR_SB_TOT + 2 * SB_TOT_SLOTS
 };
 
 struct alignas(16) HotPk { float px, py, pz; unsigned tl; };
@@ -127,6 +129,7 @@
     msl_surfel *newSurfels;
     unsigned *blockSums, *blockUpd, *delList, *srcOf;
     unsigned *sbKeys, *deal;
+    SubBound *bounds;
     int dealG;
     unsigned *tickets;
     unsigned *delU;
@@ -262,6 +265,7 @@
 void map_launch_select_write(hipStream_t st, const SfDev &P, int mode, int arg, msl_surfel *out, int markDeleted);
 void map_launch_collect_changed(hipStream_t st, const SfDev &P, int ref, long long n, unsigned *count, unsigned *idxOut, msl_surfel *recOut, unsigned capOut);
 void map_launch_empty(hipStream_t st, int grid, hipEvent_t a, hipEvent_t b);
-
-}
-}
+hipError_t map_invalidate_bounds(hipStream_t st, const SfDev &P);
+
+}
+}
diff --git a/manhattanslam_amd/csrc/msl_sf_bound.h b/manhattanslam_amd/csrc/msl_sf_bound.h
--- /dev/null
+++ b/manhattanslam_amd/csrc/msl_sf_bound.h
@@ -0,0 +1,71 @@
+#pragma once
+
+#include <math.h>
+
+#if defined(__HIPCC__)
+#define MSL_SB_HD __host__ __device__
+#else
+#define MSL_SB_HD
+#endif
+
+namespace msl {
+namespace sf {
+
+struct alignas(32) SubBound { float lo[3], hi[3]; unsigned flags, _spare; };
+constexpr unsigned SB_DIRTY = 1u, SB_YOUNG = 2u, SB_VISIT = 0xFFFFFFFFu;
+
+struct SbView { float fx, fy, cx, cy, fuseNear, fuseFar; int W, H; };
+
+enum { SB_NEAR = 1, SB_FAR = 2, SB_LEFT = 4, SB_RIGHT = 8, SB_TOP = 16, SB_BOTTOM = 32 };
+
+constexpr float SB_REL = 9.5367431640625e-07f;
+constexpr float SB_MARGIN_PX = 2.0f;
+
+#if defined(__HIP_DEVICE_COMPILE__)
+#define SB_AFTER(v, dep) asm volatile("" : "+v"(v) : "v"(dep))
+#else
+#define SB_AFTER(v, dep) ((void)0)
+#endif
+MSL_SB_HD inline void sb_row(const float *inv, const int r, float &x, float y, float z, float &p, float &s) {
+    const float a = inv[r] * x;
+    SB_AFTER(y, a);
+    const float b = inv[3 + r] * y;
+    SB_AFTER(z, b);
+    const float c = inv[6 + r] * z;
+    float d = inv[9 + r] * 1.0f;
+    SB_AFTER(d, c);
+    SB_AFTER(x, c);
+    p = ((a + b) + c) + d;
+    s = ((fabsf(a) + fabsf(b)) + fabsf(c)) + fabsf(d);
+}
+MSL_SB_HD inline unsigned sb_corner_outside(const float *inv, const SbView &V, float x, float y, float z) {
+    float p[3], s[3];
+    sb_row(inv, 0, x, y, z, p[0], s[0]); sb_row(inv, 1, x, y, z, p[1], s[1]); sb_row(inv, 2, x, y, z, p[2], s[2]);
+    unsigned m = 0;
+    const float ez = SB_REL * s[2];
+    if (p[2] + ez < V.fuseNear) m |= SB_NEAR;
+    if (p[2] - ez > V.fuseFar) m |= SB_FAR;
+    if (V.fuseNear > 0.0f) {
+        const float kl = V.cx - (0.5f - SB_MARGIN_PX), kr = V.cx - ((float)V.W - 1.5f + SB_MARGIN_PX);
+        const float kt = V.cy - (0.5f - SB_MARGIN_PX), kb = V.cy - ((float)V.H - 1.5f + SB_MARGIN_PX);
+        const float ax = fabsf(V.fx) * s[0], ay = fabsf(V.fy) * s[1];
+        const float gx = V.fx * p[0], gy = V.fy * p[1];
+        if ((gx + kl * p[2]) + SB_REL * (ax + fabsf(kl) * s[2]) < 0.0f) m |= SB_LEFT;
+        if ((gx + kr * p[2]) - SB_REL * (ax + fabsf(kr) * s[2]) > 0.0f) m |= SB_RIGHT;
+        if ((gy + kt * p[2]) + SB_REL * (ay + fabsf(kt) * s[2]) < 0.0f) m |= SB_TOP;
+        if ((gy + kb * p[2]) - SB_REL * (ay + fabsf(kb) * s[2]) > 0.0f) m |= SB_BOTTOM;
+    }
+    return m;
+}
+MSL_SB_HD inline unsigned sb_box_corner_outside(const float *inv, const SbView &V, const float lo[3], const float hi[3], unsigned c) {
+    return sb_corner_outside(inv, V, (c & 1u) ? hi[0] : lo[0], (c & 2u) ? hi[1] : lo[1], (c & 4u) ? hi[2] : lo[2]);
+}
+MSL_SB_HD inline bool sb_box_skippable(const float *inv, const SbView &V, const SubBound &b) {
+    if (b.flags & (SB_DIRTY | SB_YOUNG)) return false;
+    unsigned all = 63u;
+    for (unsigned c = 0; c < 8u; c++) all &= sb_box_corner_outside(inv, V, b.lo, b.hi, c);
+    return all != 0u;
+}
+
+}
+}
diff --git a/manhattanslam_amd/csrc/msl_sf_compact.hip b/manhattanslam_amd/csrc/msl_sf_compact.hip
--- a/manhattanslam_amd/csrc/msl_sf_compact.hip
+++ b/manhattanslam_amd/csrc/msl_sf_compact.hip
@@ -122,13 +122,14 @@
     msl_surfel *newSurfels;
     unsigned *blockSums, *blockUpd, *delList, *srcOf, *tickets, *delU, *delUCount;
     const unsigned *sbKeys; unsigned *deal;
+    SubBound *bounds;
 };
 __host__ inline CompactArgs compact_args(const SfDev &P, int slot) {
     CompactArgs A;
     A.nseeds = P.nseeds; A.flagStride = P.flagStride; A.dealG = P.dealG; A._pad = 0; A.cap = P.cap; A.map = P.map; A.ctr = P.ctr;
     A.candOk = P.candOk + (size_t)slot * P.flagStride; A.fused = P.fused + (size_t)slot * P.flagStride; A.cand = P.cand + (size_t)slot * P.nseeds;
     A.newSurfels = P.newSurfels; A.blockSums = P.blockSums; A.blockUpd = P.blockUpd; A.delList = P.delList; A.srcOf = P.srcOf; A.tickets = P.tickets;
-    A.delU = P.delU; A.delUCount = P.delUCount; A.sbKeys = P.sbKeys; A.deal = P.deal;
+    A.delU = P.delU; A.delUCount = P.delUCount; A.sbKeys = P.sbKeys; A.deal = P.deal; A.bounds = P.bounds;
     return A;
 }
 
@@ -306,12 +307,16 @@
     const long long nAfter = mode == 1 ? n : (D >= K ? n - (D - K) : n + (K - D));
     const bool place = mode == 0 && !bad && (unsigned long long)nAfter <= P.cap;
     auto DL = [&](long long j) -> unsigned { return single ? s_dl[j] : ld_agent(&P.delList[j]); };
+    auto touch = [&](long long slot) { P.bounds[slot / SUB_ITEMS].flags = SB_VISIT; };
     if (cnt) {
         auto emit_one = [&](const msl_surfel &e) {
             const long long k = pos++;
             P.newSurfels[k] = e;
-            if (place)
-                store_surfel(P.map, k < D ? (long long)DL(D - 1 - k) : n + (k - D), e);
+            if (place) {
+                const long long at = k < D ? (long long)DL(D - 1 - k) : n + (k - D);
+                store_surfel(P.map, at, e);
+                touch(at);
+            }
         };
         for (unsigned long long m = emit; m; m &= m - 1) emit_one(cand[s0 + __builtin_ctzll(m)]);
         for (unsigned long long mh = emitHi; mh; mh &= mh - 1) emit_one(cand[s0 + 64 + __builtin_ctzll(mh)]);
@@ -350,10 +355,10 @@
             if (threadIdx.x == 0)
                 for (long long i = 1; i <= R; i++) {
                     const long long hole = DL(R - i), src = n - i;
-                    if (src != hole) move_surfel(P.map, hole, src);
+                    if (src != hole) { move_surfel(P.map, hole, src); touch(hole); }
                 }
         } else {
-            for (long long a = t0; a < cntLow; a += stride) move_surfel(P.map, (long long)DL(a), (long long)P.srcOf[a]);
+            for (long long a = t0; a < cntLow; a += stride) { const long long d = (long long)DL(a); move_surfel(P.map, d, (long long)P.srcOf[a]); touch(d); }
         }
     }
     if (threadIdx.x == 0) { P.ctr[CTR_LIVE] = nAfter; *P.delUCount = 0; }
diff --git a/manhattanslam_amd/csrc/msl_sf_debug.hip b/manhattanslam_amd/csrc/msl_sf_debug.hip
--- a/manhattanslam_amd/csrc/msl_sf_debug.hip
+++ b/manhattanslam_amd/csrc/msl_sf_debug.hip
@@ -40,7 +40,27 @@
 }
 int msl_sf_debug_scratch(msl_sf *h, int which, size_t offset_words, uint32_t *out, size_t n_words) noexcept {
     try {
-    if (!h || !out || which < 0 || which > 5) return MSL_ERR_INVALID;
+    if (!h || !out || which < 0 || which > 7) return MSL_ERR_INVALID;
+    if (which == 7) {
+        if (n_words < 4) return MSL_ERR_INVALID;
+        MSL_HIP_TRY(hipSetDevice(h->device));
+        int rc = sync_all(h);
+        if (rc != MSL_OK) return rc;
+        std::vector<unsigned long long> tot(2 * SB_TOT_SLOTS);
+        MSL_HIP_TRY(hipMemcpy(tot.data(), h->dev.ctr + CTR_SB_TOT, sizeof(unsigned long long) * tot.size(), hipMemcpyDeviceToHost));
+        unsigned long long v = 0, s = 0;
+        for (int i = 0; i < SB_TOT_SLOTS; i++) { v += tot[2 * i]; s += tot[2 * i + 1]; }
+        out[0] = (uint32_t)v; out[1] = (uint32_t)(v >> 32); out[2] = (uint32_t)s; out[3] = (uint32_t)(s >> 32);
+        return MSL_OK;
+    }
+    if (which == 6) {
+        if (offset_words + n_words > h->blkStride * (sizeof(SubBound) / 4)) return MSL_ERR_INVALID;
+        MSL_HIP_TRY(hipSetDevice(h->device));
+        int rc = sync_all(h);
+        if (rc != MSL_OK) return rc;
+        MSL_HIP_TRY(hipMemcpy(out, reinterpret_cast<const uint32_t *>(h->dev.bounds) + offset_words, sizeof(uint32_t) * n_words, hipMemcpyDeviceToHost));
+        return MSL_OK;
+    }
     if (which == 5) {
         if (n_words < 2) return MSL_ERR_INVALID;
         out[0] = (uint32_t)h->kfClassic; out[1] = (uint32_t)h->kfDeferred;
diff --git a/manhattanslam_amd/csrc/msl_sf_fuse.hip b/manhattanslam_amd/csrc/msl_sf_fuse.hip
--- a/manhattanslam_amd/csrc/msl_sf_fuse.hip
+++ b/manhattanslam_amd/csrc/msl_sf_fuse.hip
@@ -57,12 +57,52 @@
         if (waveIdx < full) { const unsigned grp = waveIdx / T, r = waveIdx % T; lin = (long long)grp * T + (r & 7u) * FUSE_CHUNK + (r >> 3); }
         sb0 = (long long)G - 1 - lin;
     }
-    for (long long it = 0;; it++) {
+    long long nLive = 0;
+    int itFirst = 0;
+    unsigned bflFirst = SB_VISIT;
+    if constexpr (!DEFER) {
+        const unsigned lane = lane0;
+        const long long sb = sb0;
+        u32x4 bw;
+        unsigned long long bw2;
+        unsigned bfl;
+        const SubBound *bp = P.bounds() + sb;
+        nLive = P.ctr[CTR_LIVE];
+        asm volatile("s_load_dwordx4 %0, %3, 0x0\n\ts_load_dwordx2 %1, %3, 0x10\n\ts_load_dword %2, %3, 0x18\n\ts_waitcnt lgkmcnt(0)"
+                     : "=&s"(bw), "=&s"(bw2), "=&s"(bfl) : "s"(bp) : "memory");
+        if (sb >= nSubHint && sb * WSPAN >= nLive) return;
+        bflFirst = bfl;
+        if (!(bflFirst & (SB_DIRTY | SB_YOUNG))) {
+            float fxv = P.fx, fyv = P.fy, cxv = P.cx, cyv = P.cy, nearv = P.fuseNear;
+            int wv = P.W, hv = P.H;
+            asm volatile("" : "+v"(fxv), "+v"(fyv), "+v"(cxv), "+v"(cyv), "+v"(wv), "+v"(hv), "+v"(nearv));
+            const SbView V = {fxv, fyv, cxv, cyv, nearv, P.fuseFar, wv, hv};
+            const float lo[3] = {__uint_as_float(bw[0]), __uint_as_float(bw[1]), __uint_as_float(bw[2])};
+            const float hi[3] = {__uint_as_float(bw[3]), __uint_as_float((unsigned)bw2), __uint_as_float((unsigned)(bw2 >> 32))};
+            float qx = (lane & 1u) ? hi[0] : lo[0], qy = (lane & 2u) ? hi[1] : lo[1], qz = (lane & 4u) ? hi[2] : lo[2];
+            asm volatile("" : "+v"(qx), "+v"(qy), "+v"(qz));
+            int m = (int)sb_corner_outside(F.inv, V, qx, qy, qz);
+            m &= __builtin_amdgcn_update_dpp(m, m, 0xB1, 0xF, 0xF, false);
+            m &= __builtin_amdgcn_update_dpp(m, m, 0x4E, 0xF, 0xF, false);
+            m &= __builtin_amdgcn_update_dpp(m, m, 0x141, 0xF, 0xF, false);
+            if (__builtin_amdgcn_readfirstlane(m) != 0) {
+                if (lane == 0) {
+                    P.sbKeys()[sb] = 255u; P.blockSums[sb] = 0u; P.blockUpd[sb] = 0u;
+                    atomicAdd(reinterpret_cast<unsigned long long *>(P.ctr + CTR_SB_TOT) + 2 * ((unsigned)sb & (SB_TOT_SLOTS - 1)) + 1, 1ull);
+                }
+                if ((sb + G) * WSPAN >= nLive) return;
+                itFirst = 1;
+            }
+        }
+    }
+    if constexpr (!DEFER) { bflFirst = (bflFirst & (SB_DIRTY | SB_YOUNG)) << 28; asm volatile("" : "+v"(bflFirst)); }
+    for (int it = itFirst;; it++) {
         unsigned lane = lane0;
         asm volatile("" : "+v"(lane));
 #define REC_LOCAL(k) (64u * (unsigned)(k) + lane)
-        const long long sb = sb0 + it * G;
+        const long long sb = sb0 + (long long)it * G;
         long long c0, n = 0, cntIdx;
+        unsigned bflags = (SB_DIRTY | SB_YOUNG) << 28;
         if (DEFER && spawnWave) {
             c0 = E0 + it * WSPAN;
             n = E0 + (long long)spK;
@@ -78,18 +118,25 @@
                     E0 = ((long long)__builtin_amdgcn_readfirstlane((int)(E0v >> 32)) << 32) | (unsigned)__builtin_amdgcn_readfirstlane((int)E0v);
                     if (c0 >= E0) return;
                 }
-            } else if (sb >= nSubHint && c0 >= __hip_atomic_load(&P.ctr[CTR_LIVE], __ATOMIC_RELAXED, __HIP_MEMORY_SCOPE_AGENT)) return;
+            } else if (DEFER) {
+                if (sb >= nSubHint && c0 >= __hip_atomic_load(&P.ctr[CTR_LIVE], __ATOMIC_RELAXED, __HIP_MEMORY_SCOPE_AGENT)) return;
+            } else {
+                n = nLive;
+                if (it > 0) { if (c0 >= n) return; }
+                else bflags = bflFirst;
+            }
         }
         HotPk hq[KPL];
 #pragma unroll
         for (int k = 0; k < KPL; k++) hq[k] = M.hot[c0 + REC_LOCAL(k)];
-        if (!pending) n = P.ctr[CTR_LIVE];
+        if (!pending) { if (DEFER) n = P.ctr[CTR_LIVE]; }
         else if (!spawnWave) {
             E0 = ((long long)__builtin_amdgcn_readfirstlane((int)(E0v >> 32)) << 32) | (unsigned)__builtin_amdgcn_readfirstlane((int)E0v);
             if (c0 >= E0) return;
             n = E0;
         }
         unsigned stp = 0;
+        if (!DEFER) stp = bflags;
         unsigned keyAcc = 0;
         float pzv[KPL];
         unsigned offT[KPL];
@@ -127,6 +174,39 @@
             stp |= (unsigned)st << (2 * k); pzv[k] = pc[2];
             offT[k] = off;
         }
+        if (!DEFER && (stp >> 28) != 0u && __ballot((stp & 0xFFFFu) != 0u) == 0ull) {
+            const unsigned bfl = (unsigned)__builtin_amdgcn_readfirstlane((int)(stp >> 28));
+            constexpr float INF = __builtin_inff();
+            bool young = false, bad = false;
+            float bl[3] = {INF, INF, INF}, bh[3] = {-INF, -INF, -INF};
+#pragma unroll
+            for (int k = 0; k < KPL; k++) {
+                const bool in = c0 + REC_LOCAL(k) < n;
+                const unsigned tl = hq[k].tl;
+                young = young || (in && (tl - (5u << 20)) >= (0x80000000u - (5u << 20)));
+                const float q[3] = {hq[k].px, hq[k].py, hq[k].pz};
+                bad = bad || (in && !((fabsf(q[0]) + fabsf(q[1])) + fabsf(q[2]) < INF));
+#pragma unroll
+                for (int a = 0; a < 3; a++) { bl[a] = fminf(bl[a], in ? q[a] : INF); bh[a] = fmaxf(bh[a], in ? q[a] : -INF); }
+            }
+            const unsigned fnew = __ballot(young) != 0ull ? SB_YOUNG : 0u;
+            if (bfl & SB_DIRTY) {
+                if (__ballot(bad) == 0ull) {
+#pragma unroll
+                    for (int a = 0; a < 3; a++)
+#pragma unroll
+                        for (int o = 32; o > 0; o >>= 1) { bl[a] = fminf(bl[a], __shfl_xor(bl[a], o)); bh[a] = fmaxf(bh[a], __shfl_xor(bh[a], o)); }
+                    if (lane == 0) {
+                        u32x4 *bq = reinterpret_cast<u32x4 *>(P.bounds() + sb);
+                        const u32x4 b0 = {__float_as_uint(bl[0]), __float_as_uint(bl[1]), __float_as_uint(bl[2]), __float_as_uint(bh[0])};
+                        const u32x4 b1 = {__float_as_uint(bh[1]), __float_as_uint(bh[2]), fnew, 0u};
+                        st16(bq, b0); st16(bq + 1, b1);
+                    }
+                }
+            } else if (fnew == 0u) {
+                if (lane == 0) P.bounds()[sb].flags = 0u;
+            }
+        }
         uint2 tx[KPL];
         {
 #pragma unroll
@@ -138,7 +218,7 @@
             const unsigned ks = (unsigned)__builtin_amdgcn_readlane((int)wave_incl_scan(keyAcc), 63);
             const unsigned kc = ks >> 16;
             const unsigned key = kc ? min((unsigned)((float)(ks & 0xFFFFu) * __builtin_amdgcn_rcpf((float)kc)), 254u) : 255u;
-            if (lane == 0) P.sbKeys[cntIdx] = key;
+            if (lane == 0) P.sbKeys()[cntIdx] = key;
         }
         unsigned fl = 0;
         unsigned cntDel = 0;
@@ -280,6 +360,10 @@
         if (lane == 0) {
             if (!DEFER) P.blockSums[cntIdx] = cntDel + cntDelB;
             P.blockUpd[cntIdx] = nupd;
+            if (!DEFER) {
+                atomicAdd(reinterpret_cast<unsigned long long *>(P.ctr + CTR_SB_TOT) + 2 * ((unsigned)sb & (SB_TOT_SLOTS - 1)), 1ull);
+                if (cntDel + cntDelB + nupd) P.bounds()[sb].flags = SB_VISIT;
+            }
         }
         if (!(DEFER && spawnWave) && (sb + G) * WSPAN >= n) return;
     }
diff --git a/manhattanslam_amd/csrc/msl_sf_map.hip b/manhattanslam_amd/csrc/msl_sf_map.hip
--- a/manhattanslam_amd/csrc/msl_sf_map.hip
+++ b/manhattanslam_amd/csrc/msl_sf_map.hip
@@ -141,5 +141,6 @@
     hipLaunchKernelGGL(k_collect_changed, dim3(nblk), dim3(64), 0, st, P, ref, n, count, idxOut, recOut, capOut);
 }
 void map_launch_empty(hipStream_t st, int grid, hipEvent_t a, hipEvent_t b) { hipExtLaunchKernelGGL(k_empty, dim3((unsigned)grid), dim3(64), 0, st, a, b, 0, grid); }
+hipError_t map_invalidate_bounds(hipStream_t st, const SfDev &P) { return hipMemsetAsync(P.bounds, 0xFF, sizeof(SubBound) * (size_t)(P.cap / SUB_ITEMS), st); }
 }
 }
diff --git a/manhattanslam_amd/csrc/msl_sf_map_dev.h b/manhattanslam_amd/csrc/msl_sf_map_dev.h
--- a/manhattanslam_amd/csrc/msl_sf_map_dev.h
+++ b/manhattanslam_amd/csrc/msl_sf_map_dev.h
@@ -123,7 +123,12 @@
     HotPk *hot; ColdRec *cold;
     long long *ctr;
     unsigned *blockSums, *blockUpd;
-    unsigned *sbKeys;
+    unsigned blkStride;
+#ifdef __HIPCC__
+    __device__ __forceinline__ size_t stride_here() const { unsigned s = blkStride; asm volatile("" : "+s"(s)); return s; }
+    __device__ __forceinline__ unsigned *sbKeys() const { return blockSums + stride_here(); }
+    __device__ __forceinline__ SubBound *bounds() const { return reinterpret_cast<SubBound *>(blockSums + 3 * stride_here()); }
+#endif
     const unsigned *deal;
     unsigned *delOut;
     unsigned *delCount;
@@ -132,7 +137,7 @@
 __host__ inline FuseArgs fuse_args(const SfDev &P, int slot, bool deferred, unsigned blkStride, bool dealt = false) {
     FuseArgs A;
     A.W = P.W; A.H = P.H; A.nseeds = P.nseeds; A.kf = P.kf; A.prevSlot = P.prevSlotAbs; A.rowScale = (254 << 16) / P.H;
-    A.sbKeys = P.sbKeys; A.deal = dealt ? P.deal : nullptr;
+    A.blkStride = blkStride; A.deal = dealt ? P.deal : nullptr;
     A.fx = P.fx; A.fy = P.fy; A.cx = P.cx; A.cy = P.cy; A.fuseFar = P.fuseFar; A.fuseNear = P.fuseNear;
     A.tex = P.tex + (size_t)slot * P.pxStride; A.fuseRec = P.fuseRec + (size_t)slot * P.nseeds * 3; A.fused = P.fused + (size_t)slot * P.flagStride;
     A.hot = P.map.hot; A.cold = P.map.cold; A.ctr = P.ctr;
diff --git a/manhattanslam_amd/csrc/msl_sf_replay.hip b/manhattanslam_amd/csrc/msl_sf_replay.hip
--- a/manhattanslam_amd/csrc/msl_sf_replay.hip
+++ b/manhattanslam_amd/csrc/msl_sf_replay.hip
@@ -326,6 +326,7 @@
     MSL_SF_LAUNCH(prof, SK_COMPACT, st, k_replay, dim3(1), dim3(64), P, F);
     hipLaunchKernelGGL(k_gather, dim3(128), dim3(256), 0, st, P);
     hipLaunchKernelGGL(k_scatter, dim3(128), dim3(256), 0, st, P);
-}
-}
-}
+    (void)map_invalidate_bounds(st, P);
+}
+}
+}
diff --git a/manhattanslam_amd/csrc/msl_sf_store.hip b/manhattanslam_amd/csrc/msl_sf_store.hip
--- a/manhattanslam_amd/csrc/msl_sf_store.hip
+++ b/manhattanslam_amd/csrc/msl_sf_store.hip
@@ -33,6 +33,7 @@
     D.cap = c;
     D.blockSums = (unsigned *)h->map.blockSums.p; D.blockUpd = (unsigned *)h->map.blockUpd.p; D.delList = (unsigned *)h->map.delList.p; D.srcOf = (unsigned *)h->map.srcOf.p;
     D.sbKeys = D.blockSums + h->blkStride; D.deal = D.blockSums + 2 * h->blkStride; D.dealG = 0;
+    D.bounds = reinterpret_cast<SubBound *>(D.blockSums + 3 * h->blkStride);
     unsigned *r = (unsigned *)h->map.rp.p;
     D.loc64 = reinterpret_cast<unsigned long long *>(r + RP_LOC64 * c);
     D.stageCold = reinterpret_cast<ColdRec *>(r + RP_STAGE_COLD * c);
@@ -97,13 +98,15 @@
     const size_t rpWords = RP_WORDS * cap + rp_bitmap_words(cap);
     msl_sf::MapBufs m;
     MSL_HIP_TRY(grow_all(h->mapStream, {{m.store, sizeof(float) * MAP_WORDS * cap},
-                                        {m.blockSums, sizeof(unsigned) * 3 * bst},
+                                        {m.blockSums, sizeof(unsigned) * 3 * bst + sizeof(SubBound) * bst},
                                         {m.blockUpd, sizeof(unsigned) * DEFER_WIN * bst},
                                         {m.delList, sizeof(unsigned) * cap}, {m.srcOf, sizeof(unsigned) * cap}, {m.rp, sizeof(unsigned) * rpWords}}));
     unsigned *nbs = (unsigned *)m.blockSums.p, *nrp = (unsigned *)m.rp.p;
     MSL_HIP_TRY(hipMemset(nbs, 0, sizeof(unsigned) * bst));
     MSL_HIP_TRY(hipMemset(nbs + bst, 0xFF, sizeof(unsigned) * bst));
     MSL_HIP_TRY(hipMemset(m.blockUpd.p, 0, sizeof(unsigned) * DEFER_WIN * bst));
+    static_assert(sizeof(SubBound) == 32 && (8200 * 3 * sizeof(unsigned)) % 32 == 0, "the bounds plane starts 32-byte aligned (cap / SUB_ITEMS is a multiple of 32)");
+    MSL_HIP_TRY(hipMemset(nbs + 3 * bst, 0xFF, sizeof(SubBound) * bst));
     MSL_HIP_TRY(hipMemset(nrp + RP_LOC64 * cap, 0, sizeof(unsigned long long) * cap));
     MSL_HIP_TRY(hipMemset(nrp + RP_VPOS_D * cap, 0, sizeof(unsigned) * cap));
     MSL_HIP_TRY(hipMemset(nrp + RP_BITMAP * cap, 0, sizeof(unsigned) * rp_bitmap_words(cap)));
@@ -163,6 +166,7 @@
 }
 
 void map_replaced(msl_sf *h, size_t n) {
+    (void)map_invalidate_bounds(h->mapStream, h->dev);
     h->liveBound = n; h->liveKnown = n; h->liveKnownKf = h->kfEnq; h->classicNext = true;
     drop_live_snapshots(h);
 }
@@ -191,6 +195,7 @@
 int map_select(msl_sf *h, const MapSelect &sel, msl_surfel *out, size_t cap, size_t *n_out, const char *what) {
     if (!h || !n_out) { set_error("%s: invalid argument", what); return MSL_ERR_INVALID; }
     if (sel.mark) { h->mirrorValid = false; h->classicNext = true; }
+    const bool marks = sel.mark;
     MSL_HIP_TRY(hipSetDevice(h->device));
     int rc = settle(h);
     if (rc != MSL_OK) return rc;
@@ -208,6 +213,7 @@
     const AosRun all{0, m};
     rc = aos_out(h, m, &sel, out, &all, 1);
     if (rc != MSL_OK) return rc;
+    if (marks) MSL_HIP_TRY(map_invalidate_bounds(s, h->dev));
     MSL_HIP_TRY(hipStreamSynchronize(s));
     return MSL_OK;
 }
diff --git a/manhattanslam_amd/csrc/msl_surfel.hip b/manhattanslam_amd/csrc/msl_surfel.hip
--- a/manhattanslam_amd/csrc/msl_surfel.hip
+++ b/manhattanslam_amd/csrc/msl_surfel.hip
@@ -319,8 +319,8 @@
     for (msl_sf::SlotSet &t : h->sets)
         for (hipEvent_t *e : {&t.pre, &t.map, &t.copy, &t.h2d}) ok = ok && hipEventCreateWithFlags(e, hipEventDisableTiming) == hipSuccess;
     const hipStream_t sm = h->mapStream;
-    ok = ok && h->d_ctr.grow(sizeof(long long) * 32, sm) == hipSuccess;
-    ok = ok && hipMemset(h->d_ctr.p, 0, sizeof(long long) * 32) == hipSuccess;
+    ok = ok && h->d_ctr.grow(sizeof(long long) * CTR_ALLOC, sm) == hipSuccess;
+    ok = ok && hipMemset(h->d_ctr.p, 0, sizeof(long long) * CTR_ALLOC) == hipSuccess;
     ok = ok && h->h_ctr.grow(sizeof(long long) * 16, sm) == hipSuccess;
     ok = ok && h->h_snap.grow(sizeof(long long) * msl_sf::NSNAP * msl_sf::SNAPW, sm) == hipSuccess;
     for (int i = 0; i < msl_sf::NSNAP && ok; i++) ok = hipEventCreateWithFlags(&h->snapEv[i], hipEventDisableTiming) == hipSuccess;
diff --git a/manhattanslam_amd/surfel.py b/manhattanslam_amd/surfel.py
--- a/manhattanslam_amd/surfel.py
+++ b/manhattanslam_amd/surfel.py
@@ -155,6 +155,15 @@
         check(lib.msl_sf_debug_scratch(self._h, int(which), int(offset), ptr(out), n_words))
         return out
 
+    def debug_bounds(self, n_subblocks, first=0):
+        w = self.debug_scratch(8 * int(n_subblocks), which=6, offset=8 * int(first)).reshape(-1, 8)
+        f = w[:, :6].copy().view(np.float32)
+        return f[:, :3], f[:, 3:6], w[:, 6].copy()
+
+    def debug_subblock_totals(self):
+        w = self.debug_scratch(4, which=7).astype(np.uint64)
+        return int(w[0] | (w[1] << np.uint64(32))), int(w[2] | (w[3] << np.uint64(32)))
+
     def debug_event_overhead(self, grid=1, n=200):
         us = C.c_float(0)
         check(lib.msl_sf_debug_event_overhead(self._h, int(grid), int(n), C.byref(us)))
```
